# aws-neuron/neuronx-distributed-training

Measured on AMD Instinct MI355X. Metric: tokens_per_sec, higher is better.
Workload: dtype bf16; 1 GPU; model=llama3-8B, global_batch=4, seq_len=8192, parallelism=tp1_zero1

## Files before the change

neuronx_distributed_training_amd/ops/csrc/bindings.cpp:

```cpp
#include <torch/extension.h>

#include <hip/hip_runtime.h>

#include <c10/hip/HIPStream.h>

extern "C" {
void launch_rmsnorm_fwd(const void*, const void*, void*, void*, long, int,
                        float, hipStream_t);
void launch_rmsnorm_bwd(const void*, const void*, const void*, const void*,
                        void*, void*, long, int, hipStream_t);
void launch_swiglu_fwd(const void*, void*, long, int, hipStream_t);
void launch_swiglu_bwd(const void*, const void*, void*, long, int,
                       hipStream_t);
void launch_rope_fwd(const void*, const void*, const void*, void*, int, int,
                     int, int, const long*, int, int, float, hipStream_t);
void launch_adamw(void*, const void*, void*, void*, const void*, const void*,
                  void*, long, float, float, float, float, float, int,
                  hipStream_t);
void launch_flash_fwd(const void*, const void*, const void*, void*, void*,
                      int, int, int, int, int, int, bool, float, int,
                      const long*, const long*, const long*, hipStream_t);
void launch_flash_fwd_dbuf(const void*, const void*, const void*, void*,
                           void*, int, int, int, int, int, int, bool, float,
                           int, const long*, const long*, const long*,
                           hipStream_t);
void launch_flash_bwd(const void*, const void*, const void*, const void*,
                      const void*, const void*, void*, void*, void*, int, int,
                      int, int, int, int, bool, float, int, const long*,
                      const long*, const long*, const long*, hipStream_t);
void launch_attn_delta(const void*, const void*, void*, int, int, int, int,
                       const long*, const long*, hipStream_t);
void launch_flash_fwd_range(const void*, const void*, const void*, void*,
                            void*, int, int, int, int, int, int, bool, float,
                            int, const long*, const long*, const long*,
                            const int*, const int*, hipStream_t);
void launch_flash_bwd_range(const void*, const void*, const void*,
                            const void*, const void*, const void*, void*,
                            void*, void*, int, int, int, int, int, int, bool,
                            float, int, const long*, const long*, const long*,
                            const long*, const int*, const int*, hipStream_t);
void launch_flash_fwd_seg(const void*, const void*, const void*, void*, void*,
                          int, int, int, int, int, float, int, const long*,
                          const long*, const long*, const int*, const int*,
                          hipStream_t);
void launch_flash_bwd_seg(const void*, const void*, const void*, const void*,
                          const void*, const void*, void*, void*, void*, int,
                          int, int, int, int, float, int, const long*,
                          const long*, const long*, const long*, const int*,
                          const int*, hipStream_t);
void launch_mfma_probe(const void*, const void*, void*, hipStream_t);
void launch_mfma_probe32(const void*, const void*, void*, hipStream_t);
void launch_flash_fwd_v3(const void*, const void*, const void*, void*, void*,
                         int, int, int, int, int, bool, float, int,
                         const long*, const long*, const long*, hipStream_t);
void launch_flash_bwd_v3(const void*, const void*, const void*, const void*,
                         const void*, const void*, void*, void*, void*, int,
                         int, int, int, int, bool, float, int, const long*,
                         const long*, const long*, const long*, hipStream_t);
void launch_moe_gemm(const void*, const void*, void*, const int*, const int*,
                     int, int, int, long, bool, hipStream_t);
void launch_moe_wgrad(const void*, const void*, void*, const int*, int, int,
                      int, hipStream_t);
void launch_ce_fwd(const void*, const void*, void*, void*, void*, long, int,
                   long, hipStream_t);
void launch_ce_bwd(const void*, const void*, const void*, const void*,
                   const void*, void*, long, int, long, hipStream_t);
}

namespace {

hipStream_t cur_stream() {
  return c10::hip::getCurrentHIPStream().stream();
}

#define CHECK_IN(t)                                             \
  TORCH_CHECK((t).is_cuda(), #t " must be on GPU");             \
  TORCH_CHECK((t).is_contiguous(), #t " must be contiguous")

std::vector<torch::Tensor> rmsnorm_fwd(torch::Tensor x, torch::Tensor w,
                                       double eps) {
  CHECK_IN(x);
  CHECK_IN(w);
  TORCH_CHECK(x.scalar_type() == torch::kBFloat16, "rmsnorm: bf16 only");
  TORCH_CHECK(w.scalar_type() == torch::kBFloat16, "rmsnorm: w must be bf16");
  auto N = x.size(0);
  auto H = x.size(1);
  TORCH_CHECK(H % 8 == 0, "hidden must be divisible by 8");
  auto y = torch::empty_like(x);
  auto invrms = torch::empty({N}, x.options().dtype(torch::kFloat32));
  launch_rmsnorm_fwd(x.data_ptr(), w.data_ptr(), y.data_ptr(),
                     invrms.data_ptr(), N, (int)H, (float)eps, cur_stream());
  return {y, invrms};
}

std::vector<torch::Tensor> rmsnorm_bwd(torch::Tensor dy, torch::Tensor x,
                                       torch::Tensor w, torch::Tensor invrms) {
  CHECK_IN(dy);
  CHECK_IN(x);
  CHECK_IN(w);
  TORCH_CHECK(w.scalar_type() == torch::kBFloat16, "rmsnorm: w must be bf16");
  auto N = x.size(0);
  auto H = x.size(1);
  auto dx = torch::empty_like(x);
  auto dw32 = torch::zeros({H}, x.options().dtype(torch::kFloat32));
  launch_rmsnorm_bwd(dy.data_ptr(), x.data_ptr(), w.data_ptr(),
                     invrms.data_ptr(), dx.data_ptr(), dw32.data_ptr(), N,
                     (int)H, cur_stream());
  return {dx, dw32.to(w.scalar_type())};
}

torch::Tensor swiglu_fwd(torch::Tensor gu) {
  CHECK_IN(gu);
  auto N = gu.size(0);
  auto I = gu.size(1) / 2;
  TORCH_CHECK(I % 8 == 0, "intermediate must be divisible by 8");
  auto y = torch::empty({N, I}, gu.options());
  launch_swiglu_fwd(gu.data_ptr(), y.data_ptr(), N, (int)I, cur_stream());
  return y;
}

torch::Tensor swiglu_bwd(torch::Tensor dy, torch::Tensor gu) {
  CHECK_IN(dy);
  CHECK_IN(gu);
  auto N = gu.size(0);
  auto I = gu.size(1) / 2;
  auto dgu = torch::empty_like(gu);
  launch_swiglu_bwd(dy.data_ptr(), gu.data_ptr(), dgu.data_ptr(), N, (int)I,
                    cur_stream());
  return dgu;
}

torch::Tensor rope_fwd(torch::Tensor x, torch::Tensor cost, torch::Tensor sint,
                       long pos_offset, long pos_offset2) {
  TORCH_CHECK(x.is_cuda() && x.dim() == 4 && x.stride(3) == 1,
              "rope: x must be [b, h, s, d] on GPU with d contiguous");
  auto cos_c = cost.contiguous();
  auto sin_c = sint.contiguous();
  TORCH_CHECK(cos_c.scalar_type() == torch::kFloat32, "rope table must be f32");
  int B = (int)x.size(0), H = (int)x.size(1), S = (int)x.size(2),
      D = (int)x.size(3);
  TORCH_CHECK(pos_offset2 < 0 || S % 2 == 0, "zigzag rope needs even s");
  auto y_mem = torch::empty({S, B, H, D}, x.options());
  long xstr[3] = {x.stride(2), x.stride(0), x.stride(1)};
  launch_rope_fwd(x.data_ptr(), cos_c.data_ptr(), sin_c.data_ptr(),
                  y_mem.data_ptr(), S, B, H, D, xstr, (int)pos_offset,
                  (int)pos_offset2, 1.0f, cur_stream());
  return y_mem.permute({1, 2, 0, 3});
}

static void check_adamw_f32(const torch::Tensor& t, const torch::Tensor& p,
                            const char* name) {
  TORCH_CHECK(t.is_cuda() && t.device() == p.device(), "adamw: ", name,
              " must be on the same GPU as p");
  TORCH_CHECK(t.scalar_type() == torch::kFloat32, "adamw: ", name,
              " must be fp32");
  TORCH_CHECK(t.is_contiguous(), "adamw: ", name, " must be contiguous");
  TORCH_CHECK(t.numel() == p.numel(), "adamw: ", name,
              " must have p's numel");
  TORCH_CHECK(reinterpret_cast<uintptr_t>(t.data_ptr()) % 16 == 0, "adamw: ",
              name, " must be 16-byte aligned");
}

void adamw_step(torch::Tensor p, torch::Tensor g, torch::Tensor m,
                torch::Tensor v, torch::Tensor wd_mask, double lr, double b1,
                double b2, double eps, double wd, long step,
                c10::optional<torch::Tensor> grad_scale,
                c10::optional<torch::Tensor> p_bf16) {
  check_adamw_f32(p, p, "p");
  check_adamw_f32(g, p, "g");
  check_adamw_f32(m, p, "m");
  check_adamw_f32(v, p, "v");
  TORCH_CHECK(wd_mask.is_cuda() && wd_mask.device() == p.device(),
              "adamw: wd_mask must be on the same GPU as p");
  TORCH_CHECK(wd_mask.scalar_type() == torch::kBool,
              "adamw: wd_mask must be bool");
  TORCH_CHECK(wd_mask.is_contiguous() && wd_mask.numel() == p.numel(),
              "adamw: wd_mask must be contiguous with p's numel");
  TORCH_CHECK(step >= 1, "adamw: step must be >= 1");
  void* gs = nullptr;
  if (grad_scale.has_value()) {
    TORCH_CHECK(grad_scale->scalar_type() == torch::kFloat32 &&
                    grad_scale->is_cuda() &&
                    grad_scale->device() == p.device(),
                "grad_scale must be a device fp32 scalar");
    TORCH_CHECK(grad_scale->numel() == 1,
                "grad_scale must have exactly one element");
    gs = grad_scale->data_ptr();
  }
  void* pb = nullptr;
  if (p_bf16.has_value()) {
    TORCH_CHECK(p_bf16->is_cuda() && p_bf16->device() == p.device(),
                "adamw: p_bf16 must be on the same GPU as p");
    TORCH_CHECK(p_bf16->scalar_type() == torch::kBFloat16 &&
                    p_bf16->is_contiguous() && p_bf16->numel() == p.numel(),
                "p_bf16 must be contiguous bf16 of the same numel");
    TORCH_CHECK(reinterpret_cast<uintptr_t>(p_bf16->data_ptr()) % 8 == 0,
                "adamw: p_bf16 must be 8-byte aligned");
    pb = p_bf16->data_ptr();
  }
  launch_adamw(p.data_ptr(), g.data_ptr(), m.data_ptr(), v.data_ptr(),
               wd_mask.data_ptr(), gs, pb, p.numel(), (float)lr, (float)b1,
               (float)b2, (float)eps, (float)wd, (int)step, cur_stream());
}

static void check_bhsd(const torch::Tensor& t, const char* name) {
  TORCH_CHECK(t.is_cuda() && t.dim() == 4 && t.stride(3) == 1,
              name, " must be [b, h, s, d] on GPU with d contiguous");
  TORCH_CHECK(t.scalar_type() == torch::kBFloat16, name, " must be bf16");
}

static torch::Tensor check_bwd_args(const torch::Tensor& q,
                                    const torch::Tensor& k,
                                    const torch::Tensor& v,
                                    const torch::Tensor& lse) {
  check_bhsd(k, "k");
  check_bhsd(v, "v");
  TORCH_CHECK(q.size(3) == 128 || q.size(3) == 64,
              "head_dim must be 64 or 128");
  TORCH_CHECK(k.size(1) > 0 && q.size(1) % k.size(1) == 0,
              "GQA head mismatch");
  TORCH_CHECK(lse.is_cuda() && lse.device() == q.device(),
              "lse must be on the same GPU as q");
  TORCH_CHECK(lse.scalar_type() == torch::kFloat32, "lse must be fp32");
  TORCH_CHECK(lse.dim() == 3 && lse.size(0) == q.size(0) &&
                  lse.size(1) == q.size(1) && lse.size(2) == q.size(2),
              "lse must have shape [B, HQ, SQ]");
  return lse.contiguous();
}

static torch::Tensor attn_delta(torch::Tensor dout, torch::Tensor o) {
  auto oc = o.stride(3) == 1 ? o : o.contiguous();
  int B = (int)dout.size(0), HQ = (int)dout.size(1), SQ = (int)dout.size(2),
      D = (int)dout.size(3);
  auto delta = torch::empty(
      {B, HQ, SQ}, dout.options().dtype(torch::kFloat32));
  long ds[3] = {dout.stride(2), dout.stride(0), dout.stride(1)};
  long os_[3] = {oc.stride(2), oc.stride(0), oc.stride(1)};
  launch_attn_delta(dout.data_ptr(), oc.data_ptr(), delta.data_ptr(), SQ, B,
                    HQ, D, ds, os_, cur_stream());
  return delta;
}

std::vector<torch::Tensor> flash_attn_fwd_v3(torch::Tensor q, torch::Tensor k,
                                             torch::Tensor v, bool causal,
                                             double scale, long window) {
  check_bhsd(q, "q");
  check_bhsd(k, "k");
  check_bhsd(v, "v");
  int B = (int)q.size(0), HQ = (int)q.size(1), S = (int)q.size(2),
      D = (int)q.size(3);
  int HKV = (int)k.size(1);
  TORCH_CHECK(D == 128 || D == 64, "head_dim must be 64 or 128");
  TORCH_CHECK(k.size(2) == S, "v3 kernel requires S_q == S_kv (use v2)");
  auto o_mem = torch::empty({S, B, HQ, D}, q.options());
  auto lse = torch::empty({B, HQ, S}, q.options().dtype(torch::kFloat32));
  long qs[3] = {q.stride(2), q.stride(0), q.stride(1)};
  long ks[3] = {k.stride(2), k.stride(0), k.stride(1)};
  long vs[3] = {v.stride(2), v.stride(0), v.stride(1)};
  launch_flash_fwd_v3(q.data_ptr(), k.data_ptr(), v.data_ptr(),
                      o_mem.data_ptr(), lse.data_ptr(), B, HQ, HKV, S, D,
                      causal, (float)scale, (int)window, qs, ks, vs,
                      cur_stream());
  return {o_mem.permute({1, 2, 0, 3}), lse};
}

std::vector<torch::Tensor> flash_attn_bwd_v3(torch::Tensor dout,
                                             torch::Tensor q, torch::Tensor k,
                                             torch::Tensor v, torch::Tensor o,
                                             torch::Tensor lse, bool causal,
                                             double scale, long window) {
  if (dout.stride(3) != 1) dout = dout.contiguous();
  check_bhsd(dout, "dout");
  check_bhsd(q, "q");
  lse = check_bwd_args(q, k, v, lse);
  int B = (int)q.size(0), HQ = (int)q.size(1), S = (int)q.size(2),
      D = (int)q.size(3);
  int HKV = (int)k.size(1);
  TORCH_CHECK(k.size(2) == S, "v3 kernel requires S_q == S_kv (use v2)");
  auto delta = attn_delta(dout, o);
  auto dq_mem = torch::empty({S, B, HQ, D}, q.options());
  int group = HQ / HKV;
  auto f32 = q.options().dtype(torch::kFloat32);
  auto dk_part = torch::empty({group, S, B, HKV, D}, f32);
  auto dv_part = torch::empty({group, S, B, HKV, D}, f32);
  long qs[3] = {q.stride(2), q.stride(0), q.stride(1)};
  long ks[3] = {k.stride(2), k.stride(0), k.stride(1)};
  long vs[3] = {v.stride(2), v.stride(0), v.stride(1)};
  long dstr[3] = {dout.stride(2), dout.stride(0), dout.stride(1)};
  launch_flash_bwd_v3(dout.data_ptr(), q.data_ptr(), k.data_ptr(),
                      v.data_ptr(), lse.data_ptr(), delta.data_ptr(),
                      dq_mem.data_ptr(), dk_part.data_ptr(),
                      dv_part.data_ptr(), B, HQ, HKV, S, D, causal,
                      (float)scale, (int)window, qs, ks, vs, dstr,
                      cur_stream());
  auto dk_mem = dk_part.sum(0).to(torch::kBFloat16);
  auto dv_mem = dv_part.sum(0).to(torch::kBFloat16);
  return {dq_mem.permute({1, 2, 0, 3}), dk_mem.permute({1, 2, 0, 3}),
          dv_mem.permute({1, 2, 0, 3})};
}

std::vector<torch::Tensor> flash_attn_fwd(torch::Tensor q, torch::Tensor k,
                                          torch::Tensor v, bool causal,
                                          double scale, long window) {
  check_bhsd(q, "q");
  check_bhsd(k, "k");
  check_bhsd(v, "v");
  int B = (int)q.size(0), HQ = (int)q.size(1), SQ = (int)q.size(2),
      D = (int)q.size(3);
  int HKV = (int)k.size(1), SKV = (int)k.size(2);
  TORCH_CHECK(D == 128 || D == 64, "head_dim must be 64 or 128");
  TORCH_CHECK(HQ % HKV == 0, "GQA head mismatch");
  TORCH_CHECK(!causal || SKV >= SQ, "causal needs S_kv >= S_q");
  auto o_mem = torch::empty({SQ, B, HQ, D}, q.options());
  auto lse = torch::empty({B, HQ, SQ}, q.options().dtype(torch::kFloat32));
  long qs[3] = {q.stride(2), q.stride(0), q.stride(1)};
  long ks[3] = {k.stride(2), k.stride(0), k.stride(1)};
  long vs[3] = {v.stride(2), v.stride(0), v.stride(1)};
  launch_flash_fwd_dbuf(q.data_ptr(), k.data_ptr(), v.data_ptr(),
                        o_mem.data_ptr(), lse.data_ptr(), B, HQ, HKV, SQ,
                        SKV, D, causal, (float)scale, (int)window, qs, ks,
                        vs, cur_stream());
  return {o_mem.permute({1, 2, 0, 3}), lse};
}

std::vector<torch::Tensor> flash_attn_fwd_sbuf(torch::Tensor q,
                                               torch::Tensor k,
                                               torch::Tensor v, bool causal,
                                               double scale, long window) {
  check_bhsd(q, "q");
  check_bhsd(k, "k");
  check_bhsd(v, "v");
  int B = (int)q.size(0), HQ = (int)q.size(1), SQ = (int)q.size(2),
      D = (int)q.size(3);
  int HKV = (int)k.size(1), SKV = (int)k.size(2);
  TORCH_CHECK(D == 128 || D == 64, "head_dim must be 64 or 128");
  TORCH_CHECK(HQ % HKV == 0, "GQA head mismatch");
  TORCH_CHECK(!causal || SKV >= SQ, "causal needs S_kv >= S_q");
  auto o_mem = torch::empty({SQ, B, HQ, D}, q.options());
  auto lse = torch::empty({B, HQ, SQ}, q.options().dtype(torch::kFloat32));
  long qs[3] = {q.stride(2), q.stride(0), q.stride(1)};
  long ks[3] = {k.stride(2), k.stride(0), k.stride(1)};
  long vs[3] = {v.stride(2), v.stride(0), v.stride(1)};
  launch_flash_fwd(q.data_ptr(), k.data_ptr(), v.data_ptr(),
                        o_mem.data_ptr(), lse.data_ptr(), B, HQ, HKV, SQ,
                        SKV, D, causal, (float)scale, (int)window, qs, ks,
                        vs, cur_stream());
  return {o_mem.permute({1, 2, 0, 3}), lse};
}

std::vector<torch::Tensor> flash_attn_bwd(torch::Tensor dout, torch::Tensor q,
                                          torch::Tensor k, torch::Tensor v,
                                          torch::Tensor o, torch::Tensor lse,
                                          bool causal, double scale,
                                          long window) {
  if (dout.stride(3) != 1) dout = dout.contiguous();
  check_bhsd(dout, "dout");
  check_bhsd(q, "q");
  lse = check_bwd_args(q, k, v, lse);
  int B = (int)q.size(0), HQ = (int)q.size(1), SQ = (int)q.size(2),
      D = (int)q.size(3);
  int HKV = (int)k.size(1), SKV = (int)k.size(2);
  TORCH_CHECK(!causal || SKV >= SQ, "causal needs S_kv >= S_q");
  auto delta = attn_delta(dout, o);
  auto dq_mem = torch::empty({SQ, B, HQ, D}, q.options());
  int group = HQ / HKV;
  auto f32 = q.options().dtype(torch::kFloat32);
  auto dk_part = torch::empty({group, SKV, B, HKV, D}, f32);
  auto dv_part = torch::empty({group, SKV, B, HKV, D}, f32);
  long qs[3] = {q.stride(2), q.stride(0), q.stride(1)};
  long ks[3] = {k.stride(2), k.stride(0), k.stride(1)};
  long vs[3] = {v.stride(2), v.stride(0), v.stride(1)};
  long ds[3] = {dout.stride(2), dout.stride(0), dout.stride(1)};
  launch_flash_bwd(dout.data_ptr(), q.data_ptr(), k.data_ptr(), v.data_ptr(),
                   lse.data_ptr(), delta.data_ptr(), dq_mem.data_ptr(),
                   dk_part.data_ptr(), dv_part.data_ptr(), B, HQ, HKV, SQ,
                   SKV, D, causal, (float)scale, (int)window, qs, ks, vs, ds,
                   cur_stream());
  auto dk_mem = dk_part.sum(0).to(torch::kBFloat16);
  auto dv_mem = dv_part.sum(0).to(torch::kBFloat16);
  return {dq_mem.permute({1, 2, 0, 3}), dk_mem.permute({1, 2, 0, 3}),
          dv_mem.permute({1, 2, 0, 3})};
}

static void check_kv_range(const torch::Tensor& t, const torch::Tensor& q,
                           const char* name) {
  TORCH_CHECK(t.is_cuda() && t.device() == q.device(), name,
              " must be on the same GPU as q");
  TORCH_CHECK(t.scalar_type() == torch::kInt, name, " must be int32");
  TORCH_CHECK(t.dim() == 1 && t.size(0) == q.size(0), name,
              " must have shape [B]");
  TORCH_CHECK(t.is_contiguous(), name, " must be contiguous");
}

std::vector<torch::Tensor> flash_attn_fwd_range(
    torch::Tensor q, torch::Tensor k, torch::Tensor v, torch::Tensor kv_lo,
    torch::Tensor kv_hi, bool causal, double scale, long window) {
  check_bhsd(q, "q");
  check_bhsd(k, "k");
  check_bhsd(v, "v");
  check_kv_range(kv_lo, q, "kv_lo");
  check_kv_range(kv_hi, q, "kv_hi");
  int B = (int)q.size(0), HQ = (int)q.size(1), SQ = (int)q.size(2),
      D = (int)q.size(3);
  int HKV = (int)k.size(1), SKV = (int)k.size(2);
  TORCH_CHECK(D == 128 || D == 64, "head_dim must be 64 or 128");
  TORCH_CHECK(HQ % HKV == 0, "GQA head mismatch");
  TORCH_CHECK(!causal || SKV >= SQ, "causal needs S_kv >= S_q");
  auto o_mem = torch::empty({SQ, B, HQ, D}, q.options());
  auto lse = torch::empty({B, HQ, SQ}, q.options().dtype(torch::kFloat32));
  long qs[3] = {q.stride(2), q.stride(0), q.stride(1)};
  long ks[3] = {k.stride(2), k.stride(0), k.stride(1)};
  long vs[3] = {v.stride(2), v.stride(0), v.stride(1)};
  launch_flash_fwd_range(q.data_ptr(), k.data_ptr(), v.data_ptr(),
                         o_mem.data_ptr(), lse.data_ptr(), B, HQ, HKV, SQ,
                         SKV, D, causal, (float)scale, (int)window, qs, ks,
                         vs, kv_lo.data_ptr<int>(), kv_hi.data_ptr<int>(),
                         cur_stream());
  return {o_mem.permute({1, 2, 0, 3}), lse};
}

std::vector<torch::Tensor> flash_attn_bwd_range(
    torch::Tensor dout, torch::Tensor q, torch::Tensor k, torch::Tensor v,
    torch::Tensor o, torch::Tensor lse, torch::Tensor kv_lo,
    torch::Tensor kv_hi, bool causal, double scale, long window) {
  if (dout.stride(3) != 1) dout = dout.contiguous();
  check_bhsd(dout, "dout");
  check_bhsd(q, "q");
  lse = check_bwd_args(q, k, v, lse);
  check_kv_range(kv_lo, q, "kv_lo");
  check_kv_range(kv_hi, q, "kv_hi");
  int B = (int)q.size(0), HQ = (int)q.size(1), SQ = (int)q.size(2),
      D = (int)q.size(3);
  int HKV = (int)k.size(1), SKV = (int)k.size(2);
  TORCH_CHECK(!causal || SKV >= SQ, "causal needs S_kv >= S_q");
  auto delta = attn_delta(dout, o);
  auto dq_mem = torch::empty({SQ, B, HQ, D}, q.options());
  int group = HQ / HKV;
  auto f32 = q.options().dtype(torch::kFloat32);
  auto dk_part = torch::empty({group, SKV, B, HKV, D}, f32);
  auto dv_part = torch::empty({group, SKV, B, HKV, D}, f32);
  long qs[3] = {q.stride(2), q.stride(0), q.stride(1)};
  long ks[3] = {k.stride(2), k.stride(0), k.stride(1)};
  long vs[3] = {v.stride(2), v.stride(0), v.stride(1)};
  long ds[3] = {dout.stride(2), dout.stride(0), dout.stride(1)};
  launch_flash_bwd_range(dout.data_ptr(), q.data_ptr(), k.data_ptr(),
                         v.data_ptr(), lse.data_ptr(), delta.data_ptr(),
                         dq_mem.data_ptr(), dk_part.data_ptr(),
                         dv_part.data_ptr(), B, HQ, HKV, SQ, SKV, D, causal,
                         (float)scale, (int)window, qs, ks, vs, ds,
                         kv_lo.data_ptr<int>(), kv_hi.data_ptr<int>(),
                         cur_stream());
  auto dk_mem = dk_part.sum(0).to(torch::kBFloat16);
  auto dv_mem = dv_part.sum(0).to(torch::kBFloat16);
  return {dq_mem.permute({1, 2, 0, 3}), dk_mem.permute({1, 2, 0, 3}),
          dv_mem.permute({1, 2, 0, 3})};
}

static void check_seg_bound(const torch::Tensor& t, const torch::Tensor& q,
                            const char* name) {
  TORCH_CHECK(t.is_cuda() && t.device() == q.device(), name,
              " must be on the same GPU as q");
  TORCH_CHECK(t.scalar_type() == torch::kInt, name, " must be int32");
  TORCH_CHECK(t.dim() == 2 && t.size(0) == q.size(0) &&
                  t.size(1) == q.size(2),
              name, " must have shape [B, S]");
  TORCH_CHECK(t.is_contiguous(), name, " must be contiguous");
}

std::vector<torch::Tensor> flash_attn_fwd_seg(
    torch::Tensor q, torch::Tensor k, torch::Tensor v, torch::Tensor q_start,
    torch::Tensor k_end, double scale, long window) {
  check_bhsd(q, "q");
  check_bhsd(k, "k");
  check_bhsd(v, "v");
  int B = (int)q.size(0), HQ = (int)q.size(1), S = (int)q.size(2),
      D = (int)q.size(3);
  int HKV = (int)k.size(1);
  TORCH_CHECK(k.size(2) == S, "segmented attention needs S_q == S_kv");
  check_seg_bound(q_start, q, "q_start");
  check_seg_bound(k_end, q, "k_end");
  TORCH_CHECK(D == 128 || D == 64, "head_dim must be 64 or 128");
  TORCH_CHECK(HQ % HKV == 0, "GQA head mismatch");
  auto o_mem = torch::empty({S, B, HQ, D}, q.options());
  auto lse = torch::empty({B, HQ, S}, q.options().dtype(torch::kFloat32));
  long qs[3] = {q.stride(2), q.stride(0), q.stride(1)};
  long ks[3] = {k.stride(2), k.stride(0), k.stride(1)};
  long vs[3] = {v.stride(2), v.stride(0), v.stride(1)};
  launch_flash_fwd_seg(q.data_ptr(), k.data_ptr(), v.data_ptr(),
                       o_mem.data_ptr(), lse.data_ptr(), B, HQ, HKV, S, D,
                       (float)scale, (int)window, qs, ks, vs,
                       q_start.data_ptr<int>(), k_end.data_ptr<int>(),
                       cur_stream());
  return {o_mem.permute({1, 2, 0, 3}), lse};
}

std::vector<torch::Tensor> flash_attn_bwd_seg(
    torch::Tensor dout, torch::Tensor q, torch::Tensor k, torch::Tensor v,
    torch::Tensor o, torch::Tensor lse, torch::Tensor q_start,
    torch::Tensor k_end, double scale, long window) {
  if (dout.stride(3) != 1) dout = dout.contiguous();
  check_bhsd(dout, "dout");
  check_bhsd(q, "q");
  lse = check_bwd_args(q, k, v, lse);
  int B = (int)q.size(0), HQ = (int)q.size(1), S = (int)q.size(2),
      D = (int)q.size(3);
  int HKV = (int)k.size(1);
  TORCH_CHECK(k.size(2) == S, "segmented attention needs S_q == S_kv");
  check_seg_bound(q_start, q, "q_start");
  check_seg_bound(k_end, q, "k_end");
  auto delta = attn_delta(dout, o);
  auto dq_mem = torch::empty({S, B, HQ, D}, q.options());
  int group = HQ / HKV;
  auto f32 = q.options().dtype(torch::kFloat32);
  auto dk_part = torch::empty({group, S, B, HKV, D}, f32);
  auto dv_part = torch::empty({group, S, B, HKV, D}, f32);
  long qs[3] = {q.stride(2), q.stride(0), q.stride(1)};
  long ks[3] = {k.stride(2), k.stride(0), k.stride(1)};
  long vs[3] = {v.stride(2), v.stride(0), v.stride(1)};
  long ds[3] = {dout.stride(2), dout.stride(0), dout.stride(1)};
  launch_flash_bwd_seg(dout.data_ptr(), q.data_ptr(), k.data_ptr(),
                       v.data_ptr(), lse.data_ptr(), delta.data_ptr(),
                       dq_mem.data_ptr(), dk_part.data_ptr(),
                       dv_part.data_ptr(), B, HQ, HKV, S, D, (float)scale,
                       (int)window, qs, ks, vs, ds, q_start.data_ptr<int>(),
                       k_end.data_ptr<int>(), cur_stream());
  auto dk_mem = dk_part.sum(0).to(torch::kBFloat16);
  auto dv_mem = dv_part.sum(0).to(torch::kBFloat16);
  return {dq_mem.permute({1, 2, 0, 3}), dk_mem.permute({1, 2, 0, 3}),
          dv_mem.permute({1, 2, 0, 3})};
}

torch::Tensor moe_gemm(torch::Tensor a, torch::Tensor w,
                       torch::Tensor tile_expert, torch::Tensor total_rows,
                       bool trans_b) {
  CHECK_IN(a);
  CHECK_IN(w);
  CHECK_IN(tile_expert);
  CHECK_IN(total_rows);
  TORCH_CHECK(a.dim() == 2, "moe_gemm: a must be [Tp, K]");
  TORCH_CHECK(w.dim() == 3, "moe_gemm: w must be [E, N, Kw]");
  TORCH_CHECK(a.scalar_type() == torch::kBFloat16 &&
                  w.scalar_type() == torch::kBFloat16,
              "moe_gemm: bf16 only");
  TORCH_CHECK(tile_expert.scalar_type() == torch::kInt &&
                  total_rows.scalar_type() == torch::kInt,
              "moe_gemm: int32 maps");
  TORCH_CHECK(w.device() == a.device() && tile_expert.device() == a.device() &&
                  total_rows.device() == a.device(),
              "moe_gemm: w and the int32 maps must be on a's device");
  TORCH_CHECK(total_rows.numel() == 1, "moe_gemm: total_rows must be [1]");
  long Tp = a.size(0);
  int K = (int)a.size(1);
  int N = (int)w.size(1), Kw = (int)w.size(2);
  TORCH_CHECK(Tp % 256 == 0, "padded rows must be a multiple of 256");
  int row_tiles = (int)(Tp / 256);
  int contraction = trans_b ? N : Kw;
  int out_cols = trans_b ? Kw : N;
  TORCH_CHECK(K == contraction, "moe_gemm: contraction mismatch");
  TORCH_CHECK(K % 8 == 0, "moe_gemm: contraction % 8");
  TORCH_CHECK(out_cols % 128 == 0, "moe_gemm: out cols % 128");
  TORCH_CHECK(tile_expert.numel() >= row_tiles,
              "moe_gemm: tile_expert shorter than Tp / 256");
  auto c = torch::empty({Tp, out_cols}, a.options());
  launch_moe_gemm(a.data_ptr(), w.data_ptr(), c.data_ptr(),
                  tile_expert.data_ptr<int>(), total_rows.data_ptr<int>(),
                  row_tiles, K, out_cols, (long)N * Kw, trans_b,
                  cur_stream());
  return c;
}

torch::Tensor moe_wgrad(torch::Tensor dy, torch::Tensor x,
                        torch::Tensor seg_start, long E) {
  CHECK_IN(dy);
  CHECK_IN(x);
  CHECK_IN(seg_start);
  TORCH_CHECK(dy.dim() == 2 && x.dim() == 2,
              "moe_wgrad: dy must be [Tp, N] and x [Tp, K]");
  TORCH_CHECK(dy.scalar_type() == torch::kBFloat16 &&
                  x.scalar_type() == torch::kBFloat16,
              "moe_wgrad: bf16 only");
  TORCH_CHECK(seg_start.scalar_type() == torch::kInt, "int32 seg bounds");
  TORCH_CHECK(x.device() == dy.device() && seg_start.device() == dy.device(),
              "moe_wgrad: x and seg_start must be on dy's device");
  TORCH_CHECK(dy.size(0) == x.size(0), "moe_wgrad: dy and x row counts differ");
  TORCH_CHECK(dy.size(0) % 32 == 0, "moe_wgrad: rows % 32");
  TORCH_CHECK(E >= 1 && seg_start.numel() == E + 1,
              "moe_wgrad: seg_start must have E + 1 entries");
  int N = (int)dy.size(1), K = (int)x.size(1);
  TORCH_CHECK(N % 128 == 0 && K % 128 == 0, "moe_wgrad: dims % 128");
  auto dw = torch::empty({E, N, K}, dy.options().dtype(torch::kFloat32));
  launch_moe_wgrad(dy.data_ptr(), x.data_ptr(), dw.data_ptr(),
                   seg_start.data_ptr<int>(), (int)E, N, K, cur_stream());
  return dw;
}

torch::Tensor mfma_probe(torch::Tensor a, torch::Tensor b) {
  CHECK_IN(a);
  CHECK_IN(b);
  auto c = torch::empty({16, 16}, a.options().dtype(torch::kFloat32));
  launch_mfma_probe(a.data_ptr(), b.data_ptr(), c.data_ptr(), cur_stream());
  return c;
}

torch::Tensor mfma_probe32(torch::Tensor a, torch::Tensor b) {
  CHECK_IN(a);
  CHECK_IN(b);
  auto c = torch::empty({32, 32}, a.options().dtype(torch::kFloat32));
  launch_mfma_probe32(a.data_ptr(), b.data_ptr(), c.data_ptr(), cur_stream());
  return c;
}

std::vector<torch::Tensor> ce_fwd(torch::Tensor logits, torch::Tensor targets,
                                  long vocab_start) {
  CHECK_IN(logits);
  TORCH_CHECK(logits.scalar_type() == torch::kBFloat16, "ce: bf16 logits");
  TORCH_CHECK(targets.scalar_type() == torch::kLong, "ce: int64 targets");
  long N = logits.size(0);
  int V = (int)logits.size(1);
  auto opt = logits.options().dtype(torch::kFloat32);
  auto row_max = torch::empty({N}, opt);
  auto row_sumexp = torch::empty({N}, opt);
  auto tgt = torch::empty({N}, opt);
  launch_ce_fwd(logits.data_ptr(), targets.contiguous().data_ptr(),
                row_max.data_ptr(), row_sumexp.data_ptr(), tgt.data_ptr(), N,
                V, vocab_start, cur_stream());
  return {row_max, row_sumexp, tgt};
}

torch::Tensor ce_bwd(torch::Tensor logits, torch::Tensor targets,
                     torch::Tensor gmax, torch::Tensor gsum,
                     torch::Tensor gout, long vocab_start) {
  CHECK_IN(logits);
  long N = logits.size(0);
  int V = (int)logits.size(1);
  auto dl = torch::empty_like(logits);
  launch_ce_bwd(logits.data_ptr(), targets.contiguous().data_ptr(),
                gmax.contiguous().data_ptr(), gsum.contiguous().data_ptr(),
                gout.contiguous().data_ptr(), dl.data_ptr(), N, V,
                vocab_start, cur_stream());
  return dl;
}

}

PYBIND11_MODULE(TORCH_EXTENSION_NAME, m) {
  m.def("rmsnorm_fwd", &rmsnorm_fwd);
  m.def("rmsnorm_bwd", &rmsnorm_bwd);
  m.def("swiglu_fwd", &swiglu_fwd);
  m.def("swiglu_bwd", &swiglu_bwd);
  m.def("rope_fwd", &rope_fwd, py::arg("x"), py::arg("cost"), py::arg("sint"),
        py::arg("pos_offset"), py::arg("pos_offset2") = -1);
  m.def("adamw_step", &adamw_step, py::arg("p"), py::arg("g"), py::arg("m"),
        py::arg("v"), py::arg("wd_mask"), py::arg("lr"), py::arg("b1"),
        py::arg("b2"), py::arg("eps"), py::arg("wd"), py::arg("step"),
        py::arg("grad_scale") = py::none(), py::arg("p_bf16") = py::none());
  m.def("flash_attn_fwd_sbuf", &flash_attn_fwd_sbuf, pybind11::arg("q"),
        pybind11::arg("k"), pybind11::arg("v"), pybind11::arg("causal"),
        pybind11::arg("scale"), pybind11::arg("window") = 0);
  m.def("flash_attn_fwd", &flash_attn_fwd, pybind11::arg("q"),
        pybind11::arg("k"), pybind11::arg("v"), pybind11::arg("causal"),
        pybind11::arg("scale"), pybind11::arg("window") = 0);
  m.def("flash_attn_bwd", &flash_attn_bwd, pybind11::arg("dout"),
        pybind11::arg("q"), pybind11::arg("k"), pybind11::arg("v"),
        pybind11::arg("o"), pybind11::arg("lse"), pybind11::arg("causal"),
        pybind11::arg("scale"), pybind11::arg("window") = 0);
  m.def("flash_attn_fwd_range", &flash_attn_fwd_range, pybind11::arg("q"),
        pybind11::arg("k"), pybind11::arg("v"), pybind11::arg("kv_lo"),
        pybind11::arg("kv_hi"), pybind11::arg("causal"),
        pybind11::arg("scale"), pybind11::arg("window") = 0);
  m.def("flash_attn_bwd_range", &flash_attn_bwd_range, pybind11::arg("dout"),
        pybind11::arg("q"), pybind11::arg("k"), pybind11::arg("v"),
        pybind11::arg("o"), pybind11::arg("lse"), pybind11::arg("kv_lo"),
        pybind11::arg("kv_hi"), pybind11::arg("causal"),
        pybind11::arg("scale"), pybind11::arg("window") = 0);
  m.def("flash_attn_fwd_seg", &flash_attn_fwd_seg, pybind11::arg("q"),
        pybind11::arg("k"), pybind11::arg("v"), pybind11::arg("q_start"),
        pybind11::arg("k_end"), pybind11::arg("scale"),
        pybind11::arg("window") = 0);
  m.def("flash_attn_bwd_seg", &flash_attn_bwd_seg, pybind11::arg("dout"),
        pybind11::arg("q"), pybind11::arg("k"), pybind11::arg("v"),
        pybind11::arg("o"), pybind11::arg("lse"), pybind11::arg("q_start"),
        pybind11::arg("k_end"), pybind11::arg("scale"),
        pybind11::arg("window") = 0);
  m.def("mfma_probe", &mfma_probe);
  m.def("mfma_probe32", &mfma_probe32);
  m.def("flash_attn_fwd_v3", &flash_attn_fwd_v3, pybind11::arg("q"),
        pybind11::arg("k"), pybind11::arg("v"), pybind11::arg("causal"),
        pybind11::arg("scale"), pybind11::arg("window") = 0);
  m.def("flash_attn_bwd_v3", &flash_attn_bwd_v3, pybind11::arg("dout"),
        pybind11::arg("q"), pybind11::arg("k"), pybind11::arg("v"),
        pybind11::arg("o"), pybind11::arg("lse"), pybind11::arg("causal"),
        pybind11::arg("scale"), pybind11::arg("window") = 0);
  m.def("ce_fwd", &ce_fwd);
  m.def("ce_bwd", &ce_bwd);
  m.def("moe_gemm", &moe_gemm);
  m.def("moe_wgrad", &moe_wgrad);
}
```

neuronx_distributed_training_amd/ops/csrc/flash_attn_bwd.hip:

```cpp
#include "attn_common.h"

template <int D, bool CAUSAL, bool RANGED = false, bool SEGMENTED = false>
__global__ __launch_bounds__(512) void flash_bwd_dkv_kernel(
    const bf16* __restrict__ dO, const bf16* __restrict__ Q,
    const bf16* __restrict__ K, const bf16* __restrict__ V,
    const float* __restrict__ LSE, const float* __restrict__ DELTA,
    float* __restrict__ dK,
    float* __restrict__ dV,
    int SQ, int SKV, int Bb, int HQ, int HKV, float scale,
    int window, long sQs, long sQb, long sQh, long sKs, long sKb, long sKh,
    long sVs, long sVb, long sVh, long sDs, long sDb, long sDh,
    const int* __restrict__ kv_lo = nullptr,
    const int* __restrict__ kv_hi = nullptr) {
  static_assert(!(RANGED && SEGMENTED), "one mask mode at a time");
  static_assert(!SEGMENTED || CAUSAL, "segments are causal");
  constexpr int BN = 256;
  constexpr int BM = 64;
  const int coff = SKV - SQ;
  constexpr int KP = D + 8;
  constexpr int VP = BM + 8;
  __shared__ __bf16 q_lds[BM * KP];
  __shared__ __bf16 do_lds[BM * KP];
  __shared__ __bf16 dot_lds[D * VP];
  __shared__ __bf16 qt_lds[D * VP];
  __shared__ __bf16 pT_lds[8 * 32 * VP];
  __shared__ __bf16 dsT_lds[8 * 32 * VP];

  const int lane = threadIdx.x & 63;
  const int wid = threadIdx.x >> 6;
  const int group = HQ / HKV;
  int kblock, bhg;
  xcd_remap(kblock, bhg);
  const int g = bhg % group;
  const int hkv = (bhg / group) % HKV;
  const int b = bhg / (group * HKV);
  int lo = 0, hi = SKV;
  if constexpr (RANGED) {
    lo = kv_lo[b];
    hi = kv_hi[b];
  }

  const bf16* Kp = K + b * sKb + hkv * sKh;
  const bf16* Vp = V + b * sVb + hkv * sVh;
  const int kbase = kblock * BN;
  const int krow_w = kbase + wid * 32;

  constexpr int DK = D / 32;
  bf16x8_t kfrag[2][DK], vfrag[2][DK];
#pragma unroll
  for (int sb = 0; sb < 2; ++sb) {
    const int r = krow_w + sb * 16 + (lane & 15);
    const long row = (r < SKV) ? r : (SKV - 1);
#pragma unroll
    for (int kk = 0; kk < DK; ++kk) {
      *(int4*)&kfrag[sb][kk] =
          *(const int4*)(Kp + row * sKs + kk * 32 + (lane >> 4) * 8);
      *(int4*)&vfrag[sb][kk] =
          *(const int4*)(Vp + row * sVs + kk * 32 + (lane >> 4) * 8);
#pragma unroll
      for (int j = 0; j < 8; ++j)
        kfrag[sb][kk][j] = (__bf16)((float)kfrag[sb][kk][j] * scale);
    }
  }

  constexpr int DN2 = D / 32;
  f32x16_t dvacc[DN2], dkacc[DN2];
#pragma unroll
  for (int nj = 0; nj < DN2; ++nj) {
    dvacc[nj] = f32x16_t{};
    dkacc[nj] = f32x16_t{};
  }

  const int wkey_min = krow_w;

  {
    const int hq = hkv * group + g;
    const bf16* Qp = Q + b * sQb + hq * sQh;
    const bf16* dOp = dO + b * sDb + hq * sDh;
    const float* Lp = LSE + ((long)b * HQ + hq) * SQ;
    const float* Dp = DELTA + ((long)b * HQ + hq) * SQ;

    const int klo = RANGED ? max(kbase, lo) : kbase;
    const int khi = RANGED ? min(kbase + BN, hi) : kbase + BN;
    const int ib0 = CAUSAL ? max(0, (klo - coff) / BM) : 0;
    int nqb = (SQ + BM - 1) / BM;
    if (CAUSAL && window > 0)
      nqb = min(nqb, (khi - 1 + window - coff + BM - 1) / BM);
    if (RANGED && klo >= khi) nqb = 0;
    const int* Sp = kv_lo + (long)b * SQ;
    if constexpr (SEGMENTED)
      nqb = min(nqb,
                (kv_hi[(long)b * SQ + min(kbase + BN, SKV) - 1] + BM - 1) / BM);
    int qs_tile_next = 0;
    if constexpr (SEGMENTED)
      if (ib0 < nqb) qs_tile_next = Sp[ib0 * BM];
    for (int ib = ib0; ib < nqb; ++ib) {
      const int qbase = ib * BM;
      const int qs_tile = qs_tile_next;
      if constexpr (SEGMENTED)
        if (ib + 1 < nqb) qs_tile_next = Sp[qbase + BM];
      {
        constexpr int KVECS = BM * D / 8;
        for (int t = threadIdx.x; t < KVECS; t += 512) {
          const int row = t / (D / 8);
          const int col8 = (t % (D / 8)) * 8;
          const int gr = qbase + row;
          int4 qv = (gr < SQ) ? *(const int4*)(Qp + (long)gr * sQs + col8)
                              : int4{0, 0, 0, 0};
          int4 dv = (gr < SQ) ? *(const int4*)(dOp + (long)gr * sDs + col8)
                              : int4{0, 0, 0, 0};
          *(int4*)&q_lds[row * KP + col8] = qv;
          *(int4*)&do_lds[row * KP + col8] = dv;
        }
        constexpr int TVECS = BM * D / 16;
        for (int t = threadIdx.x; t < TVECS; t += 512) {
          const int row = (t / (D / 8)) * 2;
          const int col8 = (t % (D / 8)) * 8;
          const int g0 = qbase + row, g1 = g0 + 1;
          int4 q0 = (g0 < SQ) ? *(const int4*)(Qp + (long)g0 * sQs + col8)
                              : int4{0, 0, 0, 0};
          int4 q1 = (g1 < SQ) ? *(const int4*)(Qp + (long)g1 * sQs + col8)
                              : int4{0, 0, 0, 0};
          int4 d0 = (g0 < SQ) ? *(const int4*)(dOp + (long)g0 * sDs + col8)
                              : int4{0, 0, 0, 0};
          int4 d1 = (g1 < SQ) ? *(const int4*)(dOp + (long)g1 * sDs + col8)
                              : int4{0, 0, 0, 0};
          const __bf16 *qe0 = (const __bf16*)&q0, *qe1 = (const __bf16*)&q1;
          const __bf16 *de0 = (const __bf16*)&d0, *de1 = (const __bf16*)&d1;
#pragma unroll
          for (int j = 0; j < 8; ++j) {
            __bf16 qp[2] = {qe0[j], qe1[j]};
            __bf16 dp[2] = {de0[j], de1[j]};
            const int r = col8 + j;
            const uint byte = tr_swz((uint)(r * VP + row) * 2, r);
            *(uint*)((char*)qt_lds + byte) = *(uint*)qp;
            *(uint*)((char*)dot_lds + byte) = *(uint*)dp;
          }
        }
      }
      __syncthreads();

      if ((!CAUSAL || wkey_min <= qbase + BM - 1 + coff) &&
          (!RANGED || (krow_w < hi && krow_w + 32 > lo)) &&
          (!SEGMENTED || krow_w + 32 > qs_tile)) {
        __bf16* pw = &pT_lds[wid * 32 * VP];
        __bf16* dw = &dsT_lds[wid * 32 * VP];
#pragma unroll
        for (int nq = 0; nq < BM / 16; ++nq) {
          f32x4_t st[2], dpt[2];
          st[0] = st[1] = f32x4_t{0.f, 0.f, 0.f, 0.f};
          dpt[0] = dpt[1] = f32x4_t{0.f, 0.f, 0.f, 0.f};
#pragma unroll
          for (int kk = 0; kk < DK; ++kk) {
            bf16x8_t qb =
                load_frag_b_rowmajorT(&q_lds[nq * 16 * KP], KP, kk * 32, lane);
            st[0] = MFMA_16x16x32(kfrag[0][kk], qb, st[0]);
            st[1] = MFMA_16x16x32(kfrag[1][kk], qb, st[1]);
            bf16x8_t db =
                load_frag_b_rowmajorT(&do_lds[nq * 16 * KP], KP, kk * 32, lane);
            dpt[0] = MFMA_16x16x32(vfrag[0][kk], db, dpt[0]);
            dpt[1] = MFMA_16x16x32(vfrag[1][kk], db, dpt[1]);
          }
          const int qcol = qbase + nq * 16 + (lane & 15);
          const float lse = (qcol < SQ) ? Lp[qcol] : 1e30f;
          const float delta = (qcol < SQ) ? Dp[qcol] : 0.f;
          int qs = 0;
          if constexpr (SEGMENTED) qs = (qcol < SQ) ? Sp[qcol] : 0;
          const bool full_patch =
              (!RANGED || (krow_w >= lo && krow_w + 31 < hi)) &&
              (!SEGMENTED || krow_w >= __builtin_amdgcn_readlane(qs, 15)) &&
              (qbase + nq * 16 + 15 < SQ) && (krow_w + 31 < SKV) &&
              (!CAUSAL || (qbase + nq * 16 + coff >= krow_w + 31)) &&
              (window <= 0 ||
               (qbase + nq * 16 + 15 + coff < krow_w + window));
          if (full_patch) {
#pragma unroll
            for (int sb = 0; sb < 2; ++sb) {
#pragma unroll
              for (int r = 0; r < 4; ++r) {
                const float p = __expf(st[sb][r] - lse);
                const float ds = p * (dpt[sb][r] - delta) * scale;
                const int lrow = sb * 16 + (lane >> 4) * 4 + r;
                pw[lrow * VP + nq * 16 + (lane & 15)] = (__bf16)p;
                dw[lrow * VP + nq * 16 + (lane & 15)] = (__bf16)ds;
              }
            }
          } else {
#pragma unroll
            for (int sb = 0; sb < 2; ++sb) {
#pragma unroll
              for (int r = 0; r < 4; ++r) {
                const int krow = krow_w + sb * 16 + (lane >> 4) * 4 + r;
                bool dead = (qcol >= SQ) || (krow >= SKV) ||
                            (CAUSAL && qcol + coff < krow);
                if (CAUSAL && window > 0)
                  dead |= (qcol + coff >= krow + window);
                if constexpr (RANGED) dead |= (krow < lo) || (krow >= hi);
                if constexpr (SEGMENTED) dead |= (krow < qs);
                const float p = dead ? 0.f : __expf(st[sb][r] - lse);
                const float ds = p * (dpt[sb][r] - delta) * scale;
                const int lrow = sb * 16 + (lane >> 4) * 4 + r;
                pw[lrow * VP + nq * 16 + (lane & 15)] = (__bf16)p;
                dw[lrow * VP + nq * 16 + (lane & 15)] = (__bf16)ds;
              }
            }
          }
        }
#pragma unroll
        for (int kq = 0; kq < BM / 16; ++kq) {
          bf16x8_t pa = load_frag_a32(pw, VP, kq * 16, lane);
          bf16x8_t da = load_frag_a32(dw, VP, kq * 16, lane);
#pragma unroll
          for (int nj = 0; nj < DN2; ++nj) {
            bf16x8_t dob =
                load_frag_b32_trT_swz(dot_lds, VP, nj * 32, kq * 16, lane);
            dvacc[nj] = MFMA_32x32x16(pa, dob, dvacc[nj]);
            bf16x8_t qb2 =
                load_frag_b32_trT_swz(qt_lds, VP, nj * 32, kq * 16, lane);
            dkacc[nj] = MFMA_32x32x16(da, qb2, dkacc[nj]);
          }
        }
      }
      __syncthreads();
    }
  }

  const long sOs = (long)Bb * HKV * D;
  const long slab = (long)g * SKV * sOs + ((long)b * HKV + hkv) * D;
  float* dKp = dK + slab;
  float* dVp = dV + slab;
#pragma unroll
  for (int nj = 0; nj < DN2; ++nj) {
#pragma unroll
    for (int r = 0; r < 16; ++r) {
      const int krow = krow_w + (r & 3) + 8 * (r >> 2) + 4 * (lane >> 5);
      if (krow < SKV) {
        const int dcol = nj * 32 + (lane & 31);
        dKp[(long)krow * sOs + dcol] = dkacc[nj][r];
        dVp[(long)krow * sOs + dcol] = dvacc[nj][r];
      }
    }
  }
}

template <int D, bool CAUSAL, int NSB, bool RANGED = false,
          bool SEGMENTED = false>
__global__ __launch_bounds__(512) void flash_bwd_dq_kernel(
    const bf16* __restrict__ dO, const bf16* __restrict__ Q,
    const bf16* __restrict__ K, const bf16* __restrict__ V,
    const float* __restrict__ LSE, const float* __restrict__ DELTA,
    bf16* __restrict__ dQ,
    int SQ, int SKV, int Bb, int HQ, int HKV, float scale, int window,
    long sQs, long sQb, long sQh, long sKs, long sKb, long sKh, long sVs,
    long sVb, long sVh, long sDs, long sDb, long sDh,
    const int* __restrict__ kv_lo = nullptr,
    const int* __restrict__ kv_hi = nullptr) {
  static_assert(!(RANGED && SEGMENTED), "one mask mode at a time");
  static_assert(!SEGMENTED || CAUSAL, "segments are causal");
  constexpr int BM = NSB * 128, BN = 64;
  const int coff = SKV - SQ;
  constexpr int KP = D + 8;
  constexpr int VP = BN + 8;
  __shared__ __bf16 k_lds[2][BN * KP];
  __shared__ __bf16 v_lds[2][BN * KP];
  __shared__ __bf16 kt_lds[2][D * VP];
  __shared__ __bf16 ds_lds[8 * NSB * 16 * VP];

  const int lane = threadIdx.x & 63;
  const int wid = threadIdx.x >> 6;
  int qblock, bh;
  xcd_remap(qblock, bh);
  const int hq = bh % HQ;
  const int b = bh / HQ;
  const int hkv = hq / (HQ / HKV);
  int lo = 0, hi = SKV;
  if constexpr (RANGED) {
    lo = kv_lo[b];
    hi = kv_hi[b];
  }

  const bf16* Qp = Q + b * sQb + hq * sQh;
  const bf16* dOp = dO + b * sDb + hq * sDh;
  const bf16* Kp = K + b * sKb + hkv * sKh;
  const bf16* Vp = V + b * sVb + hkv * sVh;
  const float* Lp = LSE + ((long)b * HQ + hq) * SQ;
  const float* Dp = DELTA + ((long)b * HQ + hq) * SQ;

  const int q0 = qblock * BM;
  const int qrow_w = q0 + wid * NSB * 16;

  constexpr int DK = D / 32;
  bf16x8_t qfrag[NSB][DK], dofrag[NSB][DK];
  float lse[NSB][4], delta[NSB][4];
  int qs[NSB][4], qs_last = 0, qs_wave = 0;
  if constexpr (SEGMENTED) {
    const int* Sp = kv_lo + (long)b * SQ;
    qs_wave = Sp[min(qrow_w, SQ - 1)];
    qs_last = Sp[min(qrow_w + NSB * 16 - 1, SQ - 1)];
#pragma unroll
    for (int sb = 0; sb < NSB; ++sb)
#pragma unroll
      for (int rr = 0; rr < 4; ++rr)
        qs[sb][rr] = Sp[min(qrow_w + sb * 16 + (lane >> 4) * 4 + rr, SQ - 1)];
  }
#pragma unroll
  for (int sb = 0; sb < NSB; ++sb) {
    const int r = qrow_w + sb * 16 + (lane & 15);
    const long row = (r < SQ) ? r : (SQ - 1);
#pragma unroll
    for (int kk = 0; kk < DK; ++kk) {
      *(int4*)&qfrag[sb][kk] =
          *(const int4*)(Qp + row * sQs + kk * 32 + (lane >> 4) * 8);
      *(int4*)&dofrag[sb][kk] =
          *(const int4*)(dOp + row * sDs + kk * 32 + (lane >> 4) * 8);
#pragma unroll
      for (int j = 0; j < 8; ++j)
        qfrag[sb][kk][j] = (__bf16)((float)qfrag[sb][kk][j] * scale);
    }
#pragma unroll
    for (int rr = 0; rr < 4; ++rr) {
      const int qrow = qrow_w + sb * 16 + (lane >> 4) * 4 + rr;
      lse[sb][rr] = (qrow < SQ) ? Lp[qrow] : 1e30f;
      delta[sb][rr] = (qrow < SQ) ? Dp[qrow] : 0.f;
    }
  }

  constexpr int DN = D / 16;
  constexpr int DN2 = D / 32;
  f32x4_t dqacc[NSB == 1 ? NSB : 1][NSB == 1 ? DN : 1];
  f32x16_t dqacc32[NSB == 2 ? DN2 : 1];
  if constexpr (NSB == 1) {
#pragma unroll
    for (int sb = 0; sb < NSB; ++sb)
#pragma unroll
      for (int nj = 0; nj < DN; ++nj)
        dqacc[sb][nj] = f32x4_t{0.f, 0.f, 0.f, 0.f};
  } else {
#pragma unroll
    for (int nj = 0; nj < DN2; ++nj) dqacc32[nj] = f32x16_t{};
  }

  int kend = CAUSAL ? min(SKV, q0 + BM + coff) : SKV;
  if constexpr (RANGED) kend = min(kend, hi);
  const int nkb = (kend + BN - 1) / BN;
  int jb0 =
      (CAUSAL && window > 0) ? max(0, (q0 + coff - window + 1) / BN) : 0;
  if constexpr (RANGED) jb0 = max(jb0, lo / BN);
  if constexpr (SEGMENTED) jb0 = max(jb0, kv_lo[(long)b * SQ + q0] / BN);
  const int wrow_max = qrow_w + NSB * 16 - 1;

  auto stage_kv = [&](int jb, int buf) {
    const int kbase = jb * BN;
    constexpr int KVECS = BN * D / 8;
    for (int t = threadIdx.x; t < KVECS; t += 512) {
      const int row = t / (D / 8);
      const int col8 = (t % (D / 8)) * 8;
      const int gr = kbase + row;
      int4 kv = (gr < SKV) ? *(const int4*)(Kp + (long)gr * sKs + col8)
                           : int4{0, 0, 0, 0};
      int4 vv = (gr < SKV) ? *(const int4*)(Vp + (long)gr * sVs + col8)
                           : int4{0, 0, 0, 0};
      *(int4*)&k_lds[buf][row * KP + col8] = kv;
      *(int4*)&v_lds[buf][row * KP + col8] = vv;
    }
    constexpr int TVECS = BN * D / 16;
    for (int t = threadIdx.x; t < TVECS; t += 512) {
      const int row = (t / (D / 8)) * 2;
      const int col8 = (t % (D / 8)) * 8;
      const int g0 = kbase + row, g1 = g0 + 1;
      int4 k0 = (g0 < SKV) ? *(const int4*)(Kp + (long)g0 * sKs + col8)
                           : int4{0, 0, 0, 0};
      int4 k1 = (g1 < SKV) ? *(const int4*)(Kp + (long)g1 * sKs + col8)
                           : int4{0, 0, 0, 0};
      const __bf16 *e0 = (const __bf16*)&k0, *e1 = (const __bf16*)&k1;
#pragma unroll
      for (int j = 0; j < 8; ++j) {
        __bf16 pr[2] = {e0[j], e1[j]};
        const int r = col8 + j;
        *(uint*)((char*)kt_lds[buf] + tr_swz((uint)(r * VP + row) * 2, r)) =
            *(uint*)pr;
      }
    }
  };

  stage_kv(jb0, jb0 & 1);
  __syncthreads();

  for (int jb = jb0; jb < nkb; ++jb) {
    const int kbase = jb * BN;
    const int cur = jb & 1;
    if (jb + 1 < nkb) stage_kv(jb + 1, cur ^ 1);

    if ((!CAUSAL || kbase <= wrow_max + coff) &&
        (!SEGMENTED || kbase + BN > qs_wave)) {
      __bf16* dsw = &ds_lds[wid * NSB * 16 * VP];
#pragma unroll
      for (int nk = 0; nk < BN / 16; ++nk) {
        f32x4_t st[NSB], dpt[NSB];
#pragma unroll
        for (int sb = 0; sb < NSB; ++sb) {
          st[sb] = f32x4_t{0.f, 0.f, 0.f, 0.f};
          dpt[sb] = f32x4_t{0.f, 0.f, 0.f, 0.f};
        }
#pragma unroll
        for (int kk = 0; kk < DK; ++kk) {
          bf16x8_t kb = load_frag_b_rowmajorT(&k_lds[cur][nk * 16 * KP],
                                              KP, kk * 32, lane);
#pragma unroll
          for (int sb = 0; sb < NSB; ++sb)
            st[sb] = MFMA_16x16x32(qfrag[sb][kk], kb, st[sb]);
          bf16x8_t vb = load_frag_b_rowmajorT(&v_lds[cur][nk * 16 * KP],
                                              KP, kk * 32, lane);
#pragma unroll
          for (int sb = 0; sb < NSB; ++sb)
            dpt[sb] = MFMA_16x16x32(dofrag[sb][kk], vb, dpt[sb]);
        }
        const int kcol = kbase + nk * 16 + (lane & 15);
        const bool full_patch =
            (!RANGED ||
             (kbase + nk * 16 >= lo && kbase + nk * 16 + 15 < hi)) &&
            (!SEGMENTED || kbase + nk * 16 >= qs_last) &&
            (kbase + nk * 16 + 15 < SKV) &&
            (!CAUSAL || (kbase + nk * 16 + 15 <= qrow_w + coff)) &&
            (window <= 0 || (kbase + nk * 16 > qrow_w + 31 + coff - window));
        if (full_patch) {
#pragma unroll
          for (int sb = 0; sb < NSB; ++sb) {
#pragma unroll
            for (int r = 0; r < 4; ++r) {
              const float p = __expf(st[sb][r] - lse[sb][r]);
              const float ds = p * (dpt[sb][r] - delta[sb][r]) * scale;
              dsw[(sb * 16 + (lane >> 4) * 4 + r) * VP + nk * 16 +
                  (lane & 15)] = (__bf16)ds;
            }
          }
        } else {
#pragma unroll
          for (int sb = 0; sb < NSB; ++sb) {
#pragma unroll
            for (int r = 0; r < 4; ++r) {
              const int qrow = qrow_w + sb * 16 + (lane >> 4) * 4 + r;
              bool dead = (kcol >= SKV) || (CAUSAL && kcol > qrow + coff);
              if (CAUSAL && window > 0)
                dead |= (kcol <= qrow + coff - window);
              if constexpr (RANGED) dead |= (kcol < lo) || (kcol >= hi);
              if constexpr (SEGMENTED) dead |= (kcol < qs[sb][r]);
              const float p = dead ? 0.f : __expf(st[sb][r] - lse[sb][r]);
              const float ds = p * (dpt[sb][r] - delta[sb][r]) * scale;
              dsw[(sb * 16 + (lane >> 4) * 4 + r) * VP + nk * 16 +
                  (lane & 15)] = (__bf16)ds;
            }
          }
        }
      }
      if constexpr (NSB == 1) {
#pragma unroll
        for (int nj = 0; nj < DN; ++nj) {
#pragma unroll
          for (int kk = 0; kk < BN / 32; ++kk) {
            bf16x8_t kb2 =
                load_frag_b_trT_swz(kt_lds[cur], VP, nj * 16, kk * 32, lane);
            bf16x8_t da = load_frag_a(dsw, VP, kk * 32, lane);
            dqacc[0][nj] = MFMA_16x16x32(da, kb2, dqacc[0][nj]);
          }
        }
      } else {
#pragma unroll
        for (int kq = 0; kq < BN / 16; ++kq) {
          bf16x8_t da = load_frag_a32(dsw, VP, kq * 16, lane);
#pragma unroll
          for (int nj = 0; nj < DN2; ++nj) {
            bf16x8_t kb2 = load_frag_b32_trT_swz(kt_lds[cur], VP, nj * 32,
                                                 kq * 16, lane);
            dqacc32[nj] = MFMA_32x32x16(da, kb2, dqacc32[nj]);
          }
        }
      }
    }
    __syncthreads();
  }

  const long sOs = (long)Bb * HQ * D;
  bf16* dQp = dQ + ((long)b * HQ + hq) * D;
  if constexpr (NSB == 1) {
#pragma unroll
    for (int nj = 0; nj < DN; ++nj)
#pragma unroll
      for (int r = 0; r < 4; ++r) {
        const int qrow = qrow_w + (lane >> 4) * 4 + r;
        if (qrow < SQ)
          dQp[(long)qrow * sOs + nj * 16 + (lane & 15)] =
              f2bf(dqacc[0][nj][r]);
      }
  } else {
#pragma unroll
    for (int nj = 0; nj < DN2; ++nj)
#pragma unroll
      for (int r = 0; r < 16; ++r) {
        const int qrow = qrow_w + (r & 3) + 8 * (r >> 2) + 4 * (lane >> 5);
        if (qrow < SQ)
          dQp[(long)qrow * sOs + nj * 32 + (lane & 31)] =
              f2bf(dqacc32[nj][r]);
      }
  }
}

template <int D>
__global__ __launch_bounds__(256) void attn_delta_kernel(
    const bf16* __restrict__ dO, const bf16* __restrict__ O,
    float* __restrict__ DELTA, int SQ, int Bb, int HQ, long sDs, long sDb,
    long sDh, long sOs, long sOb, long sOh) {
  const int lane = threadIdx.x & 63;
  const long row = ((long)blockIdx.x * 4 + (threadIdx.x >> 6));
  const long total = (long)SQ * Bb * HQ;
  if (row >= total) return;
  const int s = (int)(row % SQ);
  const int h = (int)((row / SQ) % HQ);
  const int b = (int)(row / ((long)SQ * HQ));
  const bf16* dp = dO + b * sDb + h * sDh + s * sDs;
  const bf16* op = O + b * sOb + h * sOh + s * sOs;
  float acc = 0.f;
#pragma unroll
  for (int j = 0; j < D / 64; ++j) {
    const int c = lane + j * 64;
    acc += bf2f(dp[c]) * bf2f(op[c]);
  }
#pragma unroll
  for (int off = 1; off < 64; off <<= 1) acc += __shfl_xor(acc, off, 64);
  if (lane == 0) DELTA[row] = acc;
}

extern "C" {
void launch_attn_delta(const void* dout, const void* o, void* delta, int SQ,
                       int B, int HQ, int D, const long* dstr,
                       const long* ostr, hipStream_t stream) {
  long total = (long)SQ * B * HQ;
  dim3 grid((unsigned)((total + 3) / 4));
  dim3 blk(256);
  if (D == 128)
    attn_delta_kernel<128><<<grid, blk, 0, stream>>>(
        (const bf16*)dout, (const bf16*)o, (float*)delta, SQ, B, HQ, dstr[0],
        dstr[1], dstr[2], ostr[0], ostr[1], ostr[2]);
  else if (D == 64)
    attn_delta_kernel<64><<<grid, blk, 0, stream>>>(
        (const bf16*)dout, (const bf16*)o, (float*)delta, SQ, B, HQ, dstr[0],
        dstr[1], dstr[2], ostr[0], ostr[1], ostr[2]);
}

void launch_flash_bwd(const void* dout, const void* q, const void* k,
                      const void* v, const void* lse, const void* delta,
                      void* dq, void* dk, void* dv, int B, int HQ, int HKV,
                      int SQ, int SKV, int D, bool causal, float scale,
                      int window, const long* qstr, const long* kstr,
                      const long* vstr, const long* dostr,
                      hipStream_t stream) {
  dim3 blk(512);
  dim3 gkv((SKV + 255) / 256, B * HQ);
  const bool small = ((long)((SQ + 255) / 256) * B * HQ) < 512;
  const int bm = small ? 128 : 256;
  dim3 gq((SQ + bm - 1) / bm, B * HQ);
#define CASE(DD, CC)                                                          \
  do {                                                                        \
    flash_bwd_dkv_kernel<DD, CC><<<gkv, blk, 0, stream>>>(                    \
        (const bf16*)dout, (const bf16*)q, (const bf16*)k, (const bf16*)v,    \
        (const float*)lse, (const float*)delta, (float*)dk, (float*)dv, SQ,  \
        SKV, B, HQ, HKV, scale, window, qstr[0], qstr[1], qstr[2], kstr[0],   \
        kstr[1],                                                              \
        kstr[2], vstr[0], vstr[1], vstr[2], dostr[0], dostr[1], dostr[2]);    \
    if (small)                                                                \
      flash_bwd_dq_kernel<DD, CC, 1><<<gq, blk, 0, stream>>>(                 \
          (const bf16*)dout, (const bf16*)q, (const bf16*)k, (const bf16*)v,  \
          (const float*)lse, (const float*)delta, (bf16*)dq, SQ, SKV, B, HQ,  \
          HKV, scale, window, qstr[0], qstr[1], qstr[2], kstr[0], kstr[1],    \
          kstr[2], vstr[0], vstr[1], vstr[2], dostr[0], dostr[1], dostr[2]);  \
    else                                                                      \
      flash_bwd_dq_kernel<DD, CC, 2><<<gq, blk, 0, stream>>>(                 \
          (const bf16*)dout, (const bf16*)q, (const bf16*)k, (const bf16*)v,  \
          (const float*)lse, (const float*)delta, (bf16*)dq, SQ, SKV, B, HQ,  \
          HKV, scale, window, qstr[0], qstr[1], qstr[2], kstr[0], kstr[1],    \
          kstr[2], vstr[0], vstr[1], vstr[2], dostr[0], dostr[1], dostr[2]);  \
  } while (0)
  if (D == 128) {
    if (causal) CASE(128, true); else CASE(128, false);
  } else if (D == 64) {
    if (causal) CASE(64, true); else CASE(64, false);
  }
#undef CASE
}

void launch_flash_bwd_range(const void* dout, const void* q, const void* k,
                      const void* v, const void* lse, const void* delta,
                      void* dq, void* dk, void* dv, int B, int HQ, int HKV,
                      int SQ, int SKV, int D, bool causal, float scale,
                      int window, const long* qstr, const long* kstr,
                      const long* vstr, const long* dostr,
                      const int* kv_lo, const int* kv_hi,
                      hipStream_t stream) {
  dim3 blk(512);
  dim3 gkv((SKV + 255) / 256, B * HQ);
  const bool small = ((long)((SQ + 255) / 256) * B * HQ) < 512;
  const int bm = small ? 128 : 256;
  dim3 gq((SQ + bm - 1) / bm, B * HQ);
#define CASE(DD, CC)                                                          \
  do {                                                                        \
    flash_bwd_dkv_kernel<DD, CC, true><<<gkv, blk, 0, stream>>>(                    \
        (const bf16*)dout, (const bf16*)q, (const bf16*)k, (const bf16*)v,    \
        (const float*)lse, (const float*)delta, (float*)dk, (float*)dv, SQ,  \
        SKV, B, HQ, HKV, scale, window, qstr[0], qstr[1], qstr[2], kstr[0],   \
        kstr[1],                                                              \
        kstr[2], vstr[0], vstr[1], vstr[2], dostr[0], dostr[1], dostr[2],     \
        kv_lo, kv_hi);                                                        \
    if (small)                                                                \
      flash_bwd_dq_kernel<DD, CC, 1, true><<<gq, blk, 0, stream>>>(                 \
          (const bf16*)dout, (const bf16*)q, (const bf16*)k, (const bf16*)v,  \
          (const float*)lse, (const float*)delta, (bf16*)dq, SQ, SKV, B, HQ,  \
          HKV, scale, window, qstr[0], qstr[1], qstr[2], kstr[0], kstr[1],    \
          kstr[2], vstr[0], vstr[1], vstr[2], dostr[0], dostr[1], dostr[2],   \
          kv_lo, kv_hi);                                                      \
    else                                                                      \
      flash_bwd_dq_kernel<DD, CC, 2, true><<<gq, blk, 0, stream>>>(                 \
          (const bf16*)dout, (const bf16*)q, (const bf16*)k, (const bf16*)v,  \
          (const float*)lse, (const float*)delta, (bf16*)dq, SQ, SKV, B, HQ,  \
          HKV, scale, window, qstr[0], qstr[1], qstr[2], kstr[0], kstr[1],    \
          kstr[2], vstr[0], vstr[1], vstr[2], dostr[0], dostr[1], dostr[2],   \
          kv_lo, kv_hi);                                                      \
  } while (0)
  if (D == 128) {
    if (causal) CASE(128, true); else CASE(128, false);
  } else if (D == 64) {
    if (causal) CASE(64, true); else CASE(64, false);
  }
#undef CASE
}

void launch_flash_bwd_seg(const void* dout, const void* q, const void* k,
                      const void* v, const void* lse, const void* delta,
                      void* dq, void* dk, void* dv, int B, int HQ, int HKV,
                      int S, int D, float scale, int window,
                      const long* qstr, const long* kstr, const long* vstr,
                      const long* dostr, const int* q_start, const int* k_end,
                      hipStream_t stream) {
  dim3 blk(512);
  dim3 gkv((S + 255) / 256, B * HQ);
  const bool small = ((long)((S + 255) / 256) * B * HQ) < 512;
  const int bm = small ? 128 : 256;
  dim3 gq((S + bm - 1) / bm, B * HQ);
#define CASE(DD)                                                              \
  do {                                                                        \
    flash_bwd_dkv_kernel<DD, true, false, true><<<gkv, blk, 0, stream>>>(     \
        (const bf16*)dout, (const bf16*)q, (const bf16*)k, (const bf16*)v,    \
        (const float*)lse, (const float*)delta, (float*)dk, (float*)dv, S,   \
        S, B, HQ, HKV, scale, window, qstr[0], qstr[1], qstr[2], kstr[0],     \
        kstr[1],                                                              \
        kstr[2], vstr[0], vstr[1], vstr[2], dostr[0], dostr[1], dostr[2],     \
        q_start, k_end);                                                      \
    if (small)                                                                \
      flash_bwd_dq_kernel<DD, true, 1, false, true>                           \
          <<<gq, blk, 0, stream>>>(                                           \
          (const bf16*)dout, (const bf16*)q, (const bf16*)k, (const bf16*)v,  \
          (const float*)lse, (const float*)delta, (bf16*)dq, S, S, B, HQ,     \
          HKV, scale, window, qstr[0], qstr[1], qstr[2], kstr[0], kstr[1],    \
          kstr[2], vstr[0], vstr[1], vstr[2], dostr[0], dostr[1], dostr[2],   \
          q_start, k_end);                                                    \
    else                                                                      \
      flash_bwd_dq_kernel<DD, true, 2, false, true>                           \
          <<<gq, blk, 0, stream>>>(                                           \
          (const bf16*)dout, (const bf16*)q, (const bf16*)k, (const bf16*)v,  \
          (const float*)lse, (const float*)delta, (bf16*)dq, S, S, B, HQ,     \
          HKV, scale, window, qstr[0], qstr[1], qstr[2], kstr[0], kstr[1],    \
          kstr[2], vstr[0], vstr[1], vstr[2], dostr[0], dostr[1], dostr[2],   \
          q_start, k_end);                                                    \
  } while (0)
  if (D == 128) CASE(128);
  else if (D == 64) CASE(64);
#undef CASE
}
}
```

neuronx_distributed_training_amd/ops/flash_attn.py:

```python

from __future__ import annotations

import math
import os

import torch

from . import kernels_for


def _attn_version() -> str:
    env = os.environ.get("NXDT_ATTN_V3", "")
    if env == "1":
        return "3"
    if env == "fwd":
        return "fwd"
    return "2"


def _fwd_fn(kern, sq=None, skv=None):
    if _attn_version() in ("3", "fwd") and (sq is None or sq == skv):
        return kern.flash_attn_fwd_v3
    return kern.flash_attn_fwd


def _bwd_fn(kern, sq=None, skv=None):
    if _attn_version() == "3" and (sq is None or sq == skv):
        return kern.flash_attn_bwd_v3
    return kern.flash_attn_bwd


def mask_to_kv_range_tensors(attention_mask):
    m = attention_mask != 0
    s = m.size(1)
    mi = m.to(torch.int32)
    has = m.any(dim=1)
    lo = torch.argmax(mi, dim=1)
    hi = s - torch.argmax(mi.flip(1), dim=1)
    zero = torch.zeros_like(lo)
    lo = torch.where(has, lo, zero)
    hi = torch.where(has, hi, zero)
    contiguous = (mi.sum(dim=1) == hi - lo).all()
    return lo.to(torch.int32), hi.to(torch.int32), contiguous


def mask_to_kv_range(attention_mask):
    lo, hi, contiguous = mask_to_kv_range_tensors(attention_mask)
    return lo, hi, bool(contiguous)


def _norm_kv_range(kv_range, b, skv, device):
    lo, hi = kv_range
    lo = torch.as_tensor(lo, device=device).to(torch.int32).reshape(-1)
    hi = torch.as_tensor(hi, device=device).to(torch.int32).reshape(-1)
    if lo.numel() != b or hi.numel() != b:
        raise ValueError(
            f"kv_range tensors must have shape [{b}], got "
            f"{tuple(lo.shape)} / {tuple(hi.shape)}"
        )
    hi = hi.clamp(0, skv)
    lo = torch.minimum(lo.clamp(0, skv), hi)
    return lo.contiguous(), hi.contiguous()


def segment_bounds(segment_ids):
    if segment_ids.dim() != 2:
        raise ValueError(
            f"segment_ids must be [B, S], got {tuple(segment_ids.shape)}"
        )
    b, s = segment_ids.shape
    pos = torch.arange(s, device=segment_ids.device, dtype=torch.int32)
    pos = pos.expand(b, s)
    new = torch.ones(b, s, dtype=torch.bool, device=segment_ids.device)
    new[:, 1:] = segment_ids[:, 1:] != segment_ids[:, :-1]
    q_start = torch.cummax(torch.where(new, pos, torch.zeros_like(pos)),
                           dim=1).values
    last = torch.ones_like(new)
    last[:, :-1] = new[:, 1:]
    end = torch.where(last, pos + 1, torch.full_like(pos, s))
    k_end = torch.cummin(end.flip(1), dim=1).values.flip(1)
    return (q_start.to(torch.int32).contiguous(),
            k_end.to(torch.int32).contiguous())


def _make_mask(sq, sk, causal, window, device, kv_lo=None, kv_hi=None,
               q_start=None):
    mask = torch.zeros(sq, sk, dtype=torch.bool, device=device)
    if causal:
        diag = sk - sq
        mask |= torch.ones(sq, sk, dtype=torch.bool, device=device).triu(
            1 + diag
        )
        if window and window > 0:
            mask |= torch.ones(sq, sk, dtype=torch.bool, device=device).tril(
                diag - window
            )
    if kv_lo is not None:
        j = torch.arange(sk, device=device)
        out = (j[None, :] < kv_lo[:, None]) | (j[None, :] >= kv_hi[:, None])
        mask = mask[None, None] | out[:, None, None, :]
    if q_start is not None:
        j = torch.arange(sk, device=device)
        out = j[None, None, :] < q_start[:, :, None]
        mask = mask[None, None] | out[:, None]
    return mask


def _ranged_softmax(s, mask):
    s = s.masked_fill(mask, float("-inf"))
    m = s.amax(dim=-1, keepdim=True)
    empty = torch.isinf(m)
    m = torch.where(empty, torch.zeros_like(m), m)
    e = torch.exp(s - m)
    l = e.sum(dim=-1, keepdim=True)
    p = e / torch.where(empty, torch.ones_like(l), l)
    lse = torch.where(empty, torch.full_like(m, -1e30), m + torch.log(l))
    return p, lse.squeeze(-1)


def _cpu_ref_fwd(q, k, v, causal, scale, window=0, kv_lo=None, kv_hi=None,
                 q_start=None):
    hq, hkv = q.size(1), k.size(1)
    if hq != hkv:
        k = k.repeat_interleave(hq // hkv, dim=1)
        v = v.repeat_interleave(hq // hkv, dim=1)
    qf, kf, vf = q.float(), k.float(), v.float()
    s = torch.matmul(qf, kf.transpose(-1, -2)) * scale
    mask = _make_mask(q.size(-2), k.size(-2), causal, window, q.device,
                      kv_lo, kv_hi, q_start)
    if kv_lo is not None:
        p, lse = _ranged_softmax(s, mask)
    else:
        s = s.masked_fill(mask, float("-inf"))
        lse = torch.logsumexp(s, dim=-1)
        p = torch.softmax(s, dim=-1)
    o = torch.matmul(p, vf)
    return o.to(q.dtype), lse


class _FlashAttnFn(torch.autograd.Function):
    @staticmethod
    def forward(ctx, q, k, v, causal: bool, scale: float, window: int = 0,
                kv_lo=None, kv_hi=None, q_start=None, k_end=None):
        kern = kernels_for(q)
        ranged = kv_lo is not None
        segmented = q_start is not None
        if kern is not None and segmented:
            o, lse = kern.flash_attn_fwd_seg(
                q, k, v, q_start, k_end, scale, window
            )
        elif kern is not None and ranged:
            o, lse = kern.flash_attn_fwd_range(
                q, k, v, kv_lo, kv_hi, causal, scale, window
            )
        elif kern is not None:
            o, lse = _fwd_fn(kern, q.size(2), k.size(2))(
                q, k, v, causal, scale, window
            )
        else:
            o, lse = _cpu_ref_fwd(q, k, v, causal, scale, window,
                                  kv_lo, kv_hi, q_start)
        if segmented:
            ctx.save_for_backward(q, k, v, o, lse, q_start, k_end)
        elif ranged:
            ctx.save_for_backward(q, k, v, o, lse, kv_lo, kv_hi)
        else:
            ctx.save_for_backward(q, k, v, o, lse)
        ctx.ranged = ranged
        ctx.segmented = segmented
        ctx.causal = causal
        ctx.scale = scale
        ctx.window = window
        return o

    @staticmethod
    def backward(ctx, do):
        kv_lo = kv_hi = q_start = k_end = None
        none7 = (None,) * 7
        if ctx.segmented:
            q, k, v, o, lse, q_start, k_end = ctx.saved_tensors
        elif ctx.ranged:
            q, k, v, o, lse, kv_lo, kv_hi = ctx.saved_tensors
        else:
            q, k, v, o, lse = ctx.saved_tensors
        kern = kernels_for(q)
        if kern is not None and ctx.segmented:
            dq, dk, dv = kern.flash_attn_bwd_seg(
                do, q, k, v, o, lse, q_start, k_end, ctx.scale, ctx.window
            )
            return (dq, dk, dv) + none7
        if kern is not None and ctx.ranged:
            dq, dk, dv = kern.flash_attn_bwd_range(
                do, q, k, v, o, lse, kv_lo, kv_hi, ctx.causal, ctx.scale,
                ctx.window,
            )
            return (dq, dk, dv) + none7
        if kern is not None:
            dq, dk, dv = _bwd_fn(kern, q.size(2), k.size(2))(
                do, q, k, v, o, lse, ctx.causal, ctx.scale, ctx.window
            )
            return (dq, dk, dv) + none7
        hq, hkv = q.size(1), k.size(1)
        g = hq // hkv
        kx = k.repeat_interleave(g, dim=1).float()
        vx = v.repeat_interleave(g, dim=1).float()
        qf, dof = q.float(), do.float()
        s = torch.matmul(qf, kx.transpose(-1, -2)) * ctx.scale
        mask = _make_mask(q.size(-2), k.size(-2), ctx.causal, ctx.window,
                          q.device, kv_lo, kv_hi, q_start)
        if ctx.ranged:
            p, _ = _ranged_softmax(s, mask)
        else:
            s = s.masked_fill(mask, float("-inf"))
            p = torch.softmax(s, dim=-1)
        dv = torch.matmul(p.transpose(-1, -2), dof)
        dp = torch.matmul(dof, vx.transpose(-1, -2))
        delta = (dof * o.float()).sum(-1, keepdim=True)
        ds = p * (dp - delta) * ctx.scale
        dq = torch.matmul(ds, kx)
        dk = torch.matmul(ds.transpose(-1, -2), qf)
        if g > 1:
            dk = dk.reshape(dk.size(0), hkv, g, dk.size(-2), dk.size(-1)).sum(2)
            dv = dv.reshape(dv.size(0), hkv, g, dv.size(-2), dv.size(-1)).sum(2)
        return (dq.to(q.dtype), dk.to(k.dtype), dv.to(v.dtype)) + none7


def flash_attn_func(
    q: torch.Tensor,
    k: torch.Tensor,
    v: torch.Tensor,
    causal: bool = True,
    scale: float | None = None,
    window: int | None = None,
    kv_range=None,
    segment_ids=None,
    seg_bounds=None,
) -> torch.Tensor:
    if scale is None:
        scale = 1.0 / math.sqrt(q.size(-1))
    if segment_ids is not None or seg_bounds is not None:
        if segment_ids is not None and seg_bounds is not None:
            raise ValueError("give segment_ids or seg_bounds, not both")
        if kv_range is not None:
            raise ValueError("segment_ids and kv_range are mutually exclusive")
        if not causal:
            raise ValueError("segment_ids needs causal=True")
        if q.size(2) != k.size(2):
            raise ValueError(
                f"segment_ids needs S_q == S_kv, got {q.size(2)} / {k.size(2)}"
            )
        if seg_bounds is None:
            seg_bounds = segment_bounds(
                torch.as_tensor(segment_ids, device=q.device)
            )
        q_start, k_end = seg_bounds
        want = (q.size(0), q.size(2))
        if tuple(q_start.shape) != want or tuple(k_end.shape) != want:
            raise ValueError(
                f"segment_ids must have shape {list(want)}, got "
                f"{tuple(q_start.shape)}"
            )
        return _FlashAttnFn.apply(
            q, k, v, True, scale, int(window or 0), None, None,
            q_start, k_end,
        )
    if kv_range is None:
        return _FlashAttnFn.apply(q, k, v, causal, scale, int(window or 0))
    kv_lo, kv_hi = _norm_kv_range(kv_range, q.size(0), k.size(2), q.device)
    return _FlashAttnFn.apply(
        q, k, v, causal, scale, int(window or 0), kv_lo, kv_hi
    )
```

neuronx_distributed_training_amd/ops/ring_attn.py:

```python

from __future__ import annotations

import math
from typing import List

import torch
import torch.distributed as dist

from ..parallel import state as ps
from .flash_attn import _FlashAttnFn, _cpu_ref_fwd, _make_mask
from . import kernels_for


def _neighbors():
    ring = ps.get_context_model_parallel_ring_ranks()
    me = ps.get_context_model_parallel_rank()
    return ring[(me + 1) % len(ring)], ring[(me - 1) % len(ring)]


def _post_shift(send_tensors, recv_buffers):
    nxt, prv = _neighbors()
    group = ps.get_context_model_parallel_group()
    ops = []
    for t in send_tensors:
        ops.append(dist.P2POp(dist.isend, t, nxt, group=group))
    for b in recv_buffers:
        ops.append(dist.P2POp(dist.irecv, b, prv, group=group))
    return dist.batch_isend_irecv(ops)


def _fwd_block(kern, q, k, v, causal, scale):
    if kern is not None:
        o, lse = kern.flash_attn_fwd(q, k, v, causal, scale)
        return o, lse
    return _cpu_ref_fwd(q, k, v, causal, scale)


def _merge_into(acc_o, acc_lse, o, lse):
    new_lse = torch.logaddexp(acc_lse, lse)
    acc_o.mul_(torch.exp(acc_lse - new_lse).unsqueeze(-1))
    acc_o.add_(o.float() * torch.exp(lse - new_lse).unsqueeze(-1))
    acc_lse.copy_(new_lse)


def _cpu_block_bwd(do, q, k, v, out, lse, causal, scale):
    hq, hkv = q.size(1), k.size(1)
    g = hq // hkv
    kx = k.repeat_interleave(g, 1).float()
    vx = v.repeat_interleave(g, 1).float()
    qf, dof = q.float(), do.float()
    s = torch.matmul(qf, kx.transpose(-1, -2)) * scale
    if causal:
        mask = _make_mask(q.size(-2), k.size(-2), True, 0, q.device)
        s = s.masked_fill(mask, float("-inf"))
    p = torch.exp(s - lse.unsqueeze(-1))
    dv = torch.matmul(p.transpose(-1, -2), dof)
    dp = torch.matmul(dof, vx.transpose(-1, -2))
    delta = (dof * out.float()).sum(-1, keepdim=True)
    ds = p * (dp - delta) * scale
    dq = torch.matmul(ds, kx)
    dk = torch.matmul(ds.transpose(-1, -2), qf)
    if g > 1:
        dk = dk.reshape(dk.size(0), hkv, g, dk.size(-2), dk.size(-1)).sum(2)
        dv = dv.reshape(dv.size(0), hkv, g, dv.size(-2), dv.size(-1)).sum(2)
    return dq.to(q.dtype), dk.to(k.dtype), dv.to(v.dtype)


def _bwd_block(kern, do, q, k, v, out, lse, causal, scale):
    if kern is not None:
        return kern.flash_attn_bwd(
            do.contiguous(), q, k, v, out, lse, causal, scale
        )
    return _cpu_block_bwd(do, q, k, v, out, lse, causal, scale)


def _ring_fwd_hop(kern, r, j, q, k_blk, v_blk, acc_o, acc_lse, scale):
    half = q.size(2) // 2
    if j == r:
        o, lse = _fwd_block(kern, q, k_blk, v_blk, True, scale)
        _merge_into(acc_o, acc_lse, o, lse)
    elif j < r:
        o, lse = _fwd_block(
            kern, q, k_blk[:, :, :half], v_blk[:, :, :half], False, scale,
        )
        _merge_into(acc_o, acc_lse, o, lse)
    else:
        o, lse = _fwd_block(kern, q[:, :, half:], k_blk, v_blk, False, scale)
        _merge_into(acc_o[:, :, half:], acc_lse[:, :, half:], o, lse)


def _ring_bwd_hop(kern, r, j, dout, q, k_blk, v_blk, out, lse, dq_acc, scale):
    half = q.size(2) // 2
    lo_only = j < r
    if j == r:
        dq_j, dk_j, dv_j = _bwd_block(
            kern, dout, q, k_blk, v_blk, out, lse, True, scale
        )
        dq_acc += dq_j
    elif j < r:
        dq_j, dk_j, dv_j = _bwd_block(
            kern, dout, q, k_blk[:, :, :half], v_blk[:, :, :half],
            out, lse, False, scale,
        )
        dq_acc += dq_j
    else:
        dq_j, dk_j, dv_j = _bwd_block(
            kern, dout[:, :, half:], q[:, :, half:], k_blk, v_blk,
            out[:, :, half:], lse[:, :, half:], False, scale,
        )
        dq_acc[:, :, half:] += dq_j
    return dk_j, dv_j, lo_only


class _RingFlashAttnFn(torch.autograd.Function):
    @staticmethod
    def forward(ctx, q, k, v, scale):
        R = ps.get_context_model_parallel_world_size()
        r = ps.get_context_model_parallel_rank()
        kern = kernels_for(q)
        s_loc = q.size(2)
        assert s_loc % 2 == 0, "zigzag CP needs an even local sequence"
        k_cur, v_cur = k.contiguous(), v.contiguous()
        k_bufs = [torch.empty_like(k_cur), torch.empty_like(k_cur)]
        v_bufs = [torch.empty_like(v_cur), torch.empty_like(v_cur)]

        acc_o = torch.zeros(q.shape, dtype=torch.float32, device=q.device)
        acc_lse = torch.full(
            (q.size(0), q.size(1), s_loc), -1e30,
            dtype=torch.float32, device=q.device,
        )
        with torch.no_grad():
            for t in range(R):
                j = (r - t) % R
                works: List = []
                if t < R - 1:
                    works = _post_shift(
                        (k_cur, v_cur), (k_bufs[t % 2], v_bufs[t % 2])
                    )
                _ring_fwd_hop(
                    kern, r, j, q, k_cur, v_cur, acc_o, acc_lse, scale
                )
                for w in works:
                    w.wait()
                if t < R - 1:
                    k_cur, v_cur = k_bufs[t % 2], v_bufs[t % 2]
            out = acc_o.to(q.dtype)
        ctx.save_for_backward(q, k, v, out, acc_lse)
        ctx.scale = scale
        return out

    @staticmethod
    def backward(ctx, dout):
        q, k, v, out, lse = ctx.saved_tensors
        scale = ctx.scale
        R = ps.get_context_model_parallel_world_size()
        r = ps.get_context_model_parallel_rank()
        kern = kernels_for(q)
        half = q.size(2) // 2
        dout = dout.contiguous()
        out = out.contiguous()
        k_cur, v_cur = k.contiguous(), v.contiguous()
        k_bufs = [torch.empty_like(k_cur), torch.empty_like(k_cur)]
        v_bufs = [torch.empty_like(v_cur), torch.empty_like(v_cur)]
        dk_cur = torch.zeros_like(k_cur)
        dv_cur = torch.zeros_like(v_cur)
        dk_buf = torch.empty_like(dk_cur)
        dv_buf = torch.empty_like(dv_cur)
        dq_acc = torch.zeros_like(q)

        acc_works: List = []
        for t in range(R):
            j = (r - t) % R
            kv_works: List = []
            if t < R - 1:
                kv_works = _post_shift(
                    (k_cur, v_cur), (k_bufs[t % 2], v_bufs[t % 2])
                )
            dk_j, dv_j, lo_only = _ring_bwd_hop(
                kern, r, j, dout, q, k_cur, v_cur, out, lse, dq_acc, scale
            )
            for w in acc_works:
                w.wait()
            if t > 0:
                dk_cur, dk_buf = dk_buf, dk_cur
                dv_cur, dv_buf = dv_buf, dv_cur
            if lo_only:
                dk_cur[:, :, :half].add_(dk_j)
                dv_cur[:, :, :half].add_(dv_j)
            else:
                dk_cur.add_(dk_j)
                dv_cur.add_(dv_j)
            acc_works = _post_shift((dk_cur, dv_cur), (dk_buf, dv_buf))
            for w in kv_works:
                w.wait()
            if t < R - 1:
                k_cur, v_cur = k_bufs[t % 2], v_bufs[t % 2]
        for w in acc_works:
            w.wait()
        return dq_acc, dk_buf, dv_buf, None


def ring_flash_attn(
    q: torch.Tensor, k: torch.Tensor, v: torch.Tensor, scale: float = None
) -> torch.Tensor:
    if scale is None:
        scale = 1.0 / math.sqrt(q.size(-1))
    if ps.get_context_model_parallel_world_size() == 1:
        return _FlashAttnFn.apply(q, k, v, True, scale)
    return _RingFlashAttnFn.apply(q, k, v, scale)
```

setup.py:

```python

import os

from setuptools import setup

os.environ.setdefault("PYTORCH_ROCM_ARCH", "gfx950")

from torch.utils.cpp_extension import BuildExtension, CUDAExtension

HERE = os.path.dirname(os.path.abspath(__file__))
CSRC = os.path.join(HERE, "neuronx_distributed_training_amd", "ops", "csrc")

sources = [
    os.path.join(CSRC, f)
    for f in (
        "bindings.cpp",
        "rmsnorm.hip",
        "swiglu.hip",
        "rope.hip",
        "adamw.hip",
        "flash_attn_fwd.hip",
        "flash_attn_fwd_dbuf.hip",
        "flash_attn_fwd_v3.hip",
        "flash_attn_bwd_v3.hip",
        "flash_attn_bwd.hip",
        "cross_entropy.hip",
        "moe_gemm.hip",
        "probe.hip",
    )
]

import pybind11
from setuptools import Extension

setup(
    name="neuronx_distributed_training_amd_ext",
    ext_modules=[
        CUDAExtension(
            name="neuronx_distributed_training_amd.ops._C",
            sources=sources,
            extra_compile_args={
                "cxx": ["-O3", "-std=c++17"],
                "nvcc": ["-O3", "-std=c++17", "--offload-arch=gfx950"],
            },
        ),
        Extension(
            name="neuronx_distributed_training_amd.data._helpers_cpp",
            sources=[
                os.path.join(
                    HERE, "neuronx_distributed_training_amd", "data",
                    "csrc_cpu", "helpers.cpp",
                )
            ],
            include_dirs=[pybind11.get_include()],
            extra_compile_args=["-O3", "-std=c++17"],
            language="c++",
        ),
    ],
    cmdclass={"build_ext": BuildExtension.with_options(use_ninja=True)},
)
```

Before: 15780 tokens/s.

## Add pipelined dK/dV flash-attention backward kernel and make it the default

Adds a new dK/dV backward kernel for v2 flash attention that software-pipelines tile loads into LDS. It builds P and dS fragments in LDS and accumulates with 32x32x16 MFMAs, reading the transposed operands with a swizzled layout. One templated kernel covers the plain, ranged and segmented variants. The bindings are consolidated into a shared helper exposing pipe and `_sbuf` variants, selected by the NXDT_ATTN_DKV env var (default pipe). The aim is to hide global-memory latency in the dK/dV pass; the cost is a new stride limit below 2^24 elements and more code to keep correct.

```diff
diff --git a/neuronx_distributed_training_amd/ops/csrc/bindings.cpp b/neuronx_distributed_training_amd/ops/csrc/bindings.cpp
--- a/neuronx_distributed_training_amd/ops/csrc/bindings.cpp
+++ b/neuronx_distributed_training_amd/ops/csrc/bindings.cpp
@@ -27,7 +27,8 @@
 void launch_flash_bwd(const void*, const void*, const void*, const void*,
                       const void*, const void*, void*, void*, void*, int, int,
                       int, int, int, int, bool, float, int, const long*,
-                      const long*, const long*, const long*, hipStream_t);
+                      const long*, const long*, const long*, bool,
+                      hipStream_t);
 void launch_attn_delta(const void*, const void*, void*, int, int, int, int,
                        const long*, const long*, hipStream_t);
 void launch_flash_fwd_range(const void*, const void*, const void*, void*,
@@ -38,7 +39,8 @@
                             const void*, const void*, const void*, void*,
                             void*, void*, int, int, int, int, int, int, bool,
                             float, int, const long*, const long*, const long*,
-                            const long*, const int*, const int*, hipStream_t);
+                            const long*, const int*, const int*, bool,
+                            hipStream_t);
 void launch_flash_fwd_seg(const void*, const void*, const void*, void*, void*,
                           int, int, int, int, int, float, int, const long*,
                           const long*, const long*, const int*, const int*,
@@ -47,7 +49,7 @@
                           const void*, const void*, void*, void*, void*, int,
                           int, int, int, int, float, int, const long*,
                           const long*, const long*, const long*, const int*,
-                          const int*, hipStream_t);
+                          const int*, bool, hipStream_t);
 void launch_mfma_probe(const void*, const void*, void*, hipStream_t);
 void launch_mfma_probe32(const void*, const void*, void*, hipStream_t);
 void launch_flash_fwd_v3(const void*, const void*, const void*, void*, void*,
@@ -348,40 +350,6 @@
   return {o_mem.permute({1, 2, 0, 3}), lse};
 }
 
-std::vector<torch::Tensor> flash_attn_bwd(torch::Tensor dout, torch::Tensor q,
-                                          torch::Tensor k, torch::Tensor v,
-                                          torch::Tensor o, torch::Tensor lse,
-                                          bool causal, double scale,
-                                          long window) {
-  if (dout.stride(3) != 1) dout = dout.contiguous();
-  check_bhsd(dout, "dout");
-  check_bhsd(q, "q");
-  lse = check_bwd_args(q, k, v, lse);
-  int B = (int)q.size(0), HQ = (int)q.size(1), SQ = (int)q.size(2),
-      D = (int)q.size(3);
-  int HKV = (int)k.size(1), SKV = (int)k.size(2);
-  TORCH_CHECK(!causal || SKV >= SQ, "causal needs S_kv >= S_q");
-  auto delta = attn_delta(dout, o);
-  auto dq_mem = torch::empty({SQ, B, HQ, D}, q.options());
-  int group = HQ / HKV;
-  auto f32 = q.options().dtype(torch::kFloat32);
-  auto dk_part = torch::empty({group, SKV, B, HKV, D}, f32);
-  auto dv_part = torch::empty({group, SKV, B, HKV, D}, f32);
-  long qs[3] = {q.stride(2), q.stride(0), q.stride(1)};
-  long ks[3] = {k.stride(2), k.stride(0), k.stride(1)};
-  long vs[3] = {v.stride(2), v.stride(0), v.stride(1)};
-  long ds[3] = {dout.stride(2), dout.stride(0), dout.stride(1)};
-  launch_flash_bwd(dout.data_ptr(), q.data_ptr(), k.data_ptr(), v.data_ptr(),
-                   lse.data_ptr(), delta.data_ptr(), dq_mem.data_ptr(),
-                   dk_part.data_ptr(), dv_part.data_ptr(), B, HQ, HKV, SQ,
-                   SKV, D, causal, (float)scale, (int)window, qs, ks, vs, ds,
-                   cur_stream());
-  auto dk_mem = dk_part.sum(0).to(torch::kBFloat16);
-  auto dv_mem = dv_part.sum(0).to(torch::kBFloat16);
-  return {dq_mem.permute({1, 2, 0, 3}), dk_mem.permute({1, 2, 0, 3}),
-          dv_mem.permute({1, 2, 0, 3})};
-}
-
 static void check_kv_range(const torch::Tensor& t, const torch::Tensor& q,
                            const char* name) {
   TORCH_CHECK(t.is_cuda() && t.device() == q.device(), name,
@@ -419,43 +387,6 @@
   return {o_mem.permute({1, 2, 0, 3}), lse};
 }
 
-std::vector<torch::Tensor> flash_attn_bwd_range(
-    torch::Tensor dout, torch::Tensor q, torch::Tensor k, torch::Tensor v,
-    torch::Tensor o, torch::Tensor lse, torch::Tensor kv_lo,
-    torch::Tensor kv_hi, bool causal, double scale, long window) {
-  if (dout.stride(3) != 1) dout = dout.contiguous();
-  check_bhsd(dout, "dout");
-  check_bhsd(q, "q");
-  lse = check_bwd_args(q, k, v, lse);
-  check_kv_range(kv_lo, q, "kv_lo");
-  check_kv_range(kv_hi, q, "kv_hi");
-  int B = (int)q.size(0), HQ = (int)q.size(1), SQ = (int)q.size(2),
-      D = (int)q.size(3);
-  int HKV = (int)k.size(1), SKV = (int)k.size(2);
-  TORCH_CHECK(!causal || SKV >= SQ, "causal needs S_kv >= S_q");
-  auto delta = attn_delta(dout, o);
-  auto dq_mem = torch::empty({SQ, B, HQ, D}, q.options());
-  int group = HQ / HKV;
-  auto f32 = q.options().dtype(torch::kFloat32);
-  auto dk_part = torch::empty({group, SKV, B, HKV, D}, f32);
-  auto dv_part = torch::empty({group, SKV, B, HKV, D}, f32);
-  long qs[3] = {q.stride(2), q.stride(0), q.stride(1)};
-  long ks[3] = {k.stride(2), k.stride(0), k.stride(1)};
-  long vs[3] = {v.stride(2), v.stride(0), v.stride(1)};
-  long ds[3] = {dout.stride(2), dout.stride(0), dout.stride(1)};
-  launch_flash_bwd_range(dout.data_ptr(), q.data_ptr(), k.data_ptr(),
-                         v.data_ptr(), lse.data_ptr(), delta.data_ptr(),
-                         dq_mem.data_ptr(), dk_part.data_ptr(),
-                         dv_part.data_ptr(), B, HQ, HKV, SQ, SKV, D, causal,
-                         (float)scale, (int)window, qs, ks, vs, ds,
-                         kv_lo.data_ptr<int>(), kv_hi.data_ptr<int>(),
-                         cur_stream());
-  auto dk_mem = dk_part.sum(0).to(torch::kBFloat16);
-  auto dv_mem = dv_part.sum(0).to(torch::kBFloat16);
-  return {dq_mem.permute({1, 2, 0, 3}), dk_mem.permute({1, 2, 0, 3}),
-          dv_mem.permute({1, 2, 0, 3})};
-}
-
 static void check_seg_bound(const torch::Tensor& t, const torch::Tensor& q,
                             const char* name) {
   TORCH_CHECK(t.is_cuda() && t.device() == q.device(), name,
@@ -494,41 +425,94 @@
   return {o_mem.permute({1, 2, 0, 3}), lse};
 }
 
-std::vector<torch::Tensor> flash_attn_bwd_seg(
-    torch::Tensor dout, torch::Tensor q, torch::Tensor k, torch::Tensor v,
-    torch::Tensor o, torch::Tensor lse, torch::Tensor q_start,
-    torch::Tensor k_end, double scale, long window) {
+static std::vector<torch::Tensor> flash_bwd_common(
+    int mode, bool pipe, torch::Tensor dout, torch::Tensor q, torch::Tensor k,
+    torch::Tensor v, torch::Tensor o, torch::Tensor lse, const torch::Tensor* a,
+    const torch::Tensor* b, bool causal, double scale, long window) {
   if (dout.stride(3) != 1) dout = dout.contiguous();
   check_bhsd(dout, "dout");
   check_bhsd(q, "q");
   lse = check_bwd_args(q, k, v, lse);
-  int B = (int)q.size(0), HQ = (int)q.size(1), S = (int)q.size(2),
+  int B = (int)q.size(0), HQ = (int)q.size(1), SQ = (int)q.size(2),
       D = (int)q.size(3);
-  int HKV = (int)k.size(1);
-  TORCH_CHECK(k.size(2) == S, "segmented attention needs S_q == S_kv");
-  check_seg_bound(q_start, q, "q_start");
-  check_seg_bound(k_end, q, "k_end");
+  int HKV = (int)k.size(1), SKV = (int)k.size(2);
+  if (mode == 1) {
+    check_kv_range(*a, q, "kv_lo");
+    check_kv_range(*b, q, "kv_hi");
+  }
+  if (mode == 2) {
+    TORCH_CHECK(SKV == SQ, "segmented attention needs S_q == S_kv");
+    check_seg_bound(*a, q, "q_start");
+    check_seg_bound(*b, q, "k_end");
+  } else {
+    TORCH_CHECK(!causal || SKV >= SQ, "causal needs S_kv >= S_q");
+  }
+  TORCH_CHECK(!pipe || (q.stride(2) >= 0 && q.stride(2) < (1L << 24) &&
+                        dout.stride(2) >= 0 && dout.stride(2) < (1L << 24)),
+              "q / dout sequence stride must be below 2^24 elements");
   auto delta = attn_delta(dout, o);
-  auto dq_mem = torch::empty({S, B, HQ, D}, q.options());
+  auto dq_mem = torch::empty({SQ, B, HQ, D}, q.options());
   int group = HQ / HKV;
   auto f32 = q.options().dtype(torch::kFloat32);
-  auto dk_part = torch::empty({group, S, B, HKV, D}, f32);
-  auto dv_part = torch::empty({group, S, B, HKV, D}, f32);
+  auto dk_part = torch::empty({group, SKV, B, HKV, D}, f32);
+  auto dv_part = torch::empty({group, SKV, B, HKV, D}, f32);
   long qs[3] = {q.stride(2), q.stride(0), q.stride(1)};
   long ks[3] = {k.stride(2), k.stride(0), k.stride(1)};
   long vs[3] = {v.stride(2), v.stride(0), v.stride(1)};
   long ds[3] = {dout.stride(2), dout.stride(0), dout.stride(1)};
-  launch_flash_bwd_seg(dout.data_ptr(), q.data_ptr(), k.data_ptr(),
-                       v.data_ptr(), lse.data_ptr(), delta.data_ptr(),
-                       dq_mem.data_ptr(), dk_part.data_ptr(),
-                       dv_part.data_ptr(), B, HQ, HKV, S, D, (float)scale,
-                       (int)window, qs, ks, vs, ds, q_start.data_ptr<int>(),
-                       k_end.data_ptr<int>(), cur_stream());
+  if (mode == 0)
+    launch_flash_bwd(dout.data_ptr(), q.data_ptr(), k.data_ptr(),
+                     v.data_ptr(), lse.data_ptr(), delta.data_ptr(),
+                     dq_mem.data_ptr(), dk_part.data_ptr(),
+                     dv_part.data_ptr(), B, HQ, HKV, SQ, SKV, D, causal,
+                     (float)scale, (int)window, qs, ks, vs, ds, pipe,
+                     cur_stream());
+  else if (mode == 1)
+    launch_flash_bwd_range(dout.data_ptr(), q.data_ptr(), k.data_ptr(),
+                           v.data_ptr(), lse.data_ptr(), delta.data_ptr(),
+                           dq_mem.data_ptr(), dk_part.data_ptr(),
+                           dv_part.data_ptr(), B, HQ, HKV, SQ, SKV, D, causal,
+                           (float)scale, (int)window, qs, ks, vs, ds,
+                           a->data_ptr<int>(), b->data_ptr<int>(), pipe,
+                           cur_stream());
+  else
+    launch_flash_bwd_seg(dout.data_ptr(), q.data_ptr(), k.data_ptr(),
+                         v.data_ptr(), lse.data_ptr(), delta.data_ptr(),
+                         dq_mem.data_ptr(), dk_part.data_ptr(),
+                         dv_part.data_ptr(), B, HQ, HKV, SQ, D, (float)scale,
+                         (int)window, qs, ks, vs, ds, a->data_ptr<int>(),
+                         b->data_ptr<int>(), pipe, cur_stream());
   auto dk_mem = dk_part.sum(0).to(torch::kBFloat16);
   auto dv_mem = dv_part.sum(0).to(torch::kBFloat16);
   return {dq_mem.permute({1, 2, 0, 3}), dk_mem.permute({1, 2, 0, 3}),
           dv_mem.permute({1, 2, 0, 3})};
 }
+
+#define BWD_BINDINGS(SUFFIX, PIPE)                                            \
+  std::vector<torch::Tensor> flash_attn_bwd##SUFFIX(                          \
+      torch::Tensor dout, torch::Tensor q, torch::Tensor k, torch::Tensor v,  \
+      torch::Tensor o, torch::Tensor lse, bool causal, double scale,          \
+      long window) {                                                          \
+    return flash_bwd_common(0, PIPE, dout, q, k, v, o, lse, nullptr, nullptr, \
+                            causal, scale, window);                           \
+  }                                                                           \
+  std::vector<torch::Tensor> flash_attn_bwd_range##SUFFIX(                    \
+      torch::Tensor dout, torch::Tensor q, torch::Tensor k, torch::Tensor v,  \
+      torch::Tensor o, torch::Tensor lse, torch::Tensor kv_lo,                \
+      torch::Tensor kv_hi, bool causal, double scale, long window) {          \
+    return flash_bwd_common(1, PIPE, dout, q, k, v, o, lse, &kv_lo, &kv_hi,   \
+                            causal, scale, window);                           \
+  }                                                                           \
+  std::vector<torch::Tensor> flash_attn_bwd_seg##SUFFIX(                      \
+      torch::Tensor dout, torch::Tensor q, torch::Tensor k, torch::Tensor v,  \
+      torch::Tensor o, torch::Tensor lse, torch::Tensor q_start,              \
+      torch::Tensor k_end, double scale, long window) {                       \
+    return flash_bwd_common(2, PIPE, dout, q, k, v, o, lse, &q_start, &k_end, \
+                            true, scale, window);                             \
+  }
+BWD_BINDINGS(, true)
+BWD_BINDINGS(_sbuf, false)
+#undef BWD_BINDINGS
 
 torch::Tensor moe_gemm(torch::Tensor a, torch::Tensor w,
                        torch::Tensor tile_expert, torch::Tensor total_rows,
@@ -682,6 +666,21 @@
         pybind11::arg("o"), pybind11::arg("lse"), pybind11::arg("q_start"),
         pybind11::arg("k_end"), pybind11::arg("scale"),
         pybind11::arg("window") = 0);
+  m.def("flash_attn_bwd_sbuf", &flash_attn_bwd_sbuf, pybind11::arg("dout"),
+        pybind11::arg("q"), pybind11::arg("k"), pybind11::arg("v"),
+        pybind11::arg("o"), pybind11::arg("lse"), pybind11::arg("causal"),
+        pybind11::arg("scale"), pybind11::arg("window") = 0);
+  m.def("flash_attn_bwd_range_sbuf", &flash_attn_bwd_range_sbuf,
+        pybind11::arg("dout"), pybind11::arg("q"), pybind11::arg("k"),
+        pybind11::arg("v"), pybind11::arg("o"), pybind11::arg("lse"),
+        pybind11::arg("kv_lo"), pybind11::arg("kv_hi"),
+        pybind11::arg("causal"), pybind11::arg("scale"),
+        pybind11::arg("window") = 0);
+  m.def("flash_attn_bwd_seg_sbuf", &flash_attn_bwd_seg_sbuf,
+        pybind11::arg("dout"), pybind11::arg("q"), pybind11::arg("k"),
+        pybind11::arg("v"), pybind11::arg("o"), pybind11::arg("lse"),
+        pybind11::arg("q_start"), pybind11::arg("k_end"),
+        pybind11::arg("scale"), pybind11::arg("window") = 0);
   m.def("mfma_probe", &mfma_probe);
   m.def("mfma_probe32", &mfma_probe32);
   m.def("flash_attn_fwd_v3", &flash_attn_fwd_v3, pybind11::arg("q"),
diff --git a/neuronx_distributed_training_amd/ops/csrc/flash_attn_bwd.hip b/neuronx_distributed_training_amd/ops/csrc/flash_attn_bwd.hip
--- a/neuronx_distributed_training_amd/ops/csrc/flash_attn_bwd.hip
+++ b/neuronx_distributed_training_amd/ops/csrc/flash_attn_bwd.hip
@@ -547,13 +547,26 @@
         dstr[1], dstr[2], ostr[0], ostr[1], ostr[2]);
 }
 
+void launch_flash_dkv_pipe(const void* dout, const void* q, const void* k,
+                           const void* v, const void* lse, const void* delta,
+                           void* dk, void* dv, int B, int HQ, int HKV, int SQ,
+                           int SKV, int D, bool causal, float scale,
+                           int window, const long* qstr, const long* kstr,
+                           const long* vstr, const long* dostr, int mode,
+                           const int* bound_a, const int* bound_b,
+                           hipStream_t stream);
+
 void launch_flash_bwd(const void* dout, const void* q, const void* k,
                       const void* v, const void* lse, const void* delta,
                       void* dq, void* dk, void* dv, int B, int HQ, int HKV,
                       int SQ, int SKV, int D, bool causal, float scale,
                       int window, const long* qstr, const long* kstr,
-                      const long* vstr, const long* dostr,
+                      const long* vstr, const long* dostr, bool pipe,
                       hipStream_t stream) {
+  if (pipe)
+    launch_flash_dkv_pipe(dout, q, k, v, lse, delta, dk, dv, B, HQ, HKV, SQ,
+                          SKV, D, causal, scale, window, qstr, kstr, vstr,
+                          dostr, 0, nullptr, nullptr, stream);
   dim3 blk(512);
   dim3 gkv((SKV + 255) / 256, B * HQ);
   const bool small = ((long)((SQ + 255) / 256) * B * HQ) < 512;
@@ -561,6 +574,7 @@
   dim3 gq((SQ + bm - 1) / bm, B * HQ);
 #define CASE(DD, CC)                                                          \
   do {                                                                        \
+    if (!pipe)                                                                \
     flash_bwd_dkv_kernel<DD, CC><<<gkv, blk, 0, stream>>>(                    \
         (const bf16*)dout, (const bf16*)q, (const bf16*)k, (const bf16*)v,    \
         (const float*)lse, (const float*)delta, (float*)dk, (float*)dv, SQ,  \
@@ -594,8 +608,12 @@
                       int SQ, int SKV, int D, bool causal, float scale,
                       int window, const long* qstr, const long* kstr,
                       const long* vstr, const long* dostr,
-                      const int* kv_lo, const int* kv_hi,
+                      const int* kv_lo, const int* kv_hi, bool pipe,
                       hipStream_t stream) {
+  if (pipe)
+    launch_flash_dkv_pipe(dout, q, k, v, lse, delta, dk, dv, B, HQ, HKV, SQ,
+                          SKV, D, causal, scale, window, qstr, kstr, vstr,
+                          dostr, 1, kv_lo, kv_hi, stream);
   dim3 blk(512);
   dim3 gkv((SKV + 255) / 256, B * HQ);
   const bool small = ((long)((SQ + 255) / 256) * B * HQ) < 512;
@@ -603,6 +621,7 @@
   dim3 gq((SQ + bm - 1) / bm, B * HQ);
 #define CASE(DD, CC)                                                          \
   do {                                                                        \
+    if (!pipe)                                                                \
     flash_bwd_dkv_kernel<DD, CC, true><<<gkv, blk, 0, stream>>>(                    \
         (const bf16*)dout, (const bf16*)q, (const bf16*)k, (const bf16*)v,    \
         (const float*)lse, (const float*)delta, (float*)dk, (float*)dv, SQ,  \
@@ -639,7 +658,11 @@
                       int S, int D, float scale, int window,
                       const long* qstr, const long* kstr, const long* vstr,
                       const long* dostr, const int* q_start, const int* k_end,
-                      hipStream_t stream) {
+                      bool pipe, hipStream_t stream) {
+  if (pipe)
+    launch_flash_dkv_pipe(dout, q, k, v, lse, delta, dk, dv, B, HQ, HKV, S, S,
+                          D, true, scale, window, qstr, kstr, vstr, dostr, 2,
+                          q_start, k_end, stream);
   dim3 blk(512);
   dim3 gkv((S + 255) / 256, B * HQ);
   const bool small = ((long)((S + 255) / 256) * B * HQ) < 512;
@@ -647,6 +670,7 @@
   dim3 gq((S + bm - 1) / bm, B * HQ);
 #define CASE(DD)                                                              \
   do {                                                                        \
+    if (!pipe)                                                                \
     flash_bwd_dkv_kernel<DD, true, false, true><<<gkv, blk, 0, stream>>>(     \
         (const bf16*)dout, (const bf16*)q, (const bf16*)k, (const bf16*)v,    \
         (const float*)lse, (const float*)delta, (float*)dk, (float*)dv, S,   \
diff --git a/neuronx_distributed_training_amd/ops/csrc/flash_attn_bwd_dkv_pipe.hip b/neuronx_distributed_training_amd/ops/csrc/flash_attn_bwd_dkv_pipe.hip
--- /dev/null
+++ b/neuronx_distributed_training_amd/ops/csrc/flash_attn_bwd_dkv_pipe.hip
@@ -0,0 +1,344 @@
+#include "attn_common.h"
+
+template <int D, bool CAUSAL, bool RANGED = false, bool SEGMENTED = false>
+__global__ __launch_bounds__(512) void flash_bwd_dkv_pipe_kernel(
+    const bf16* __restrict__ dO, const bf16* __restrict__ Q,
+    const bf16* __restrict__ K, const bf16* __restrict__ V,
+    const float* __restrict__ LSE, const float* __restrict__ DELTA,
+    float* __restrict__ dK,
+    float* __restrict__ dV,
+    int SQ, int SKV, int Bb, int HQ, int HKV, float scale,
+    int window, long sQs, long sQb, long sQh, long sKs, long sKb, long sKh,
+    long sVs, long sVb, long sVh, long sDs, long sDb, long sDh,
+    const int* __restrict__ kv_lo = nullptr,
+    const int* __restrict__ kv_hi = nullptr) {
+  static_assert(!(RANGED && SEGMENTED), "one mask mode at a time");
+  static_assert(!SEGMENTED || CAUSAL, "segments are causal");
+  constexpr int BN = 256;
+  constexpr int BM = 64;
+  const int coff = SKV - SQ;
+  constexpr int KP = D + 8;
+  constexpr int VP = BM + 8;
+  __shared__ __attribute__((aligned(16))) __bf16 qdo_lds[2 * BM * KP];
+  __shared__ __attribute__((aligned(16))) __bf16 tr_lds[2 * D * VP];
+  __shared__ __attribute__((aligned(16))) __bf16 pds_lds[2 * 8 * 32 * VP];
+  __bf16* const q_lds = qdo_lds;
+  __bf16* const do_lds = qdo_lds + BM * KP;
+  __bf16* const dot_lds = tr_lds;
+  __bf16* const qt_lds = tr_lds + D * VP;
+  __bf16* const pT_lds = pds_lds;
+  __bf16* const dsT_lds = pds_lds + 8 * 32 * VP;
+  constexpr int PARK = (D == 128) ? 2 : 0;
+  __shared__ __attribute__((aligned(16))) __bf16 park_lds[PARK * 512 * 8 + 8];
+  __shared__ __attribute__((aligned(16))) float row_lds[3 * BM];
+
+  const int lane = threadIdx.x & 63;
+  const int wid = __builtin_amdgcn_readfirstlane(threadIdx.x >> 6);
+  const int group = HQ / HKV;
+  int kblock, bhg;
+  xcd_remap(kblock, bhg);
+  const int g = bhg % group;
+  const int hkv = (bhg / group) % HKV;
+  const int b = bhg / (group * HKV);
+  int lo = 0, hi = SKV;
+  if constexpr (RANGED) {
+    lo = kv_lo[b];
+    hi = kv_hi[b];
+  }
+
+  const bf16* Kp = K + b * sKb + hkv * sKh;
+  const bf16* Vp = V + b * sVb + hkv * sVh;
+  const int kbase = kblock * BN;
+  const int krow_w = kbase + wid * 32;
+
+  constexpr int DK = D / 32;
+  bf16x8_t kfrag[2][DK], vfrag[2][DK];
+#pragma unroll
+  for (int sb = 0; sb < 2; ++sb) {
+    const int r = krow_w + sb * 16 + (lane & 15);
+    const long row = (r < SKV) ? r : (SKV - 1);
+#pragma unroll
+    for (int kk = 0; kk < DK; ++kk) {
+      *(int4*)&kfrag[sb][kk] =
+          *(const int4*)(Kp + row * sKs + kk * 32 + (lane >> 4) * 8);
+      *(int4*)&vfrag[sb][kk] =
+          *(const int4*)(Vp + row * sVs + kk * 32 + (lane >> 4) * 8);
+#pragma unroll
+      for (int j = 0; j < 8; ++j)
+        kfrag[sb][kk][j] = (__bf16)((float)kfrag[sb][kk][j] * scale);
+    }
+  }
+
+#pragma unroll
+  for (int i = 0; i < PARK; ++i)
+    *(bf16x8_t*)&park_lds[(i * 512 + threadIdx.x) * 8] =
+        vfrag[1][DK - PARK + i];
+
+  constexpr int DN2 = D / 32;
+  f32x16_t dvacc[DN2], dkacc[DN2];
+#pragma unroll
+  for (int nj = 0; nj < DN2; ++nj) {
+    dvacc[nj] = f32x16_t{};
+    dkacc[nj] = f32x16_t{};
+  }
+
+  {
+    const int hq = hkv * group + g;
+    const bf16* Qp = Q + b * sQb + hq * sQh;
+    const bf16* dOp = dO + b * sDb + hq * sDh;
+    const float* Lp = LSE + ((long)b * HQ + hq) * SQ;
+    const float* Dp = DELTA + ((long)b * HQ + hq) * SQ;
+
+    const int klo = RANGED ? max(kbase, lo) : kbase;
+    const int khi = RANGED ? min(kbase + BN, hi) : kbase + BN;
+    const int ib0 = CAUSAL ? max(0, (klo - coff) / BM) : 0;
+    int nqb = (SQ + BM - 1) / BM;
+    if (CAUSAL && window > 0)
+      nqb = min(nqb, (khi - 1 + window - coff + BM - 1) / BM);
+    if (RANGED && klo >= khi) nqb = 0;
+    const int* Sp = kv_lo + (long)b * SQ;
+    if constexpr (SEGMENTED)
+      nqb = min(nqb,
+                (kv_hi[(long)b * SQ + min(kbase + BN, SKV) - 1] + BM - 1) / BM);
+
+    constexpr int C8 = D / 8;
+    const uint qrs = (uint)sQs * 2, dors = (uint)sDs * 2;
+    constexpr int NROWC = SEGMENTED ? 3 : 2;
+    const float* rowp = wid == 0 ? Lp : wid == 1 ? Dp : (const float*)Sp;
+
+    typedef int i32x4_t __attribute__((ext_vector_type(4)));
+    i32x4_t q0 = {0, 0, 0, 0}, q1 = q0, d0 = q0, d1 = q0;
+    float rowc = 0.f;
+    auto issue_tile = [&](int ib) {
+      const int qbase = ib * BM;
+      int t = threadIdx.x;
+      asm volatile("" : "+v"(t));
+      const int last = SQ - 1 - qbase;
+      if ((D == 128) || wid < 4) {
+        const int srow = (t / C8) * 2, scol = (t % C8) * 8;
+        const int r0 = min(srow, last), r1 = min(srow + 1, last);
+        const char* qt = (const char*)(Qp + (long)qbase * sQs);
+        const char* dt = (const char*)(dOp + (long)qbase * sDs);
+        q0 = *(const i32x4_t*)(qt + ((uint)r0 * qrs + scol * 2));
+        d0 = *(const i32x4_t*)(dt + ((uint)r0 * dors + scol * 2));
+        q1 = *(const i32x4_t*)(qt + ((uint)r1 * qrs + scol * 2));
+        d1 = *(const i32x4_t*)(dt + ((uint)r1 * dors + scol * 2));
+      }
+      if (wid < NROWC)
+        rowc = *(const float*)((const char*)(rowp + qbase) +
+                               (uint)min(t & 63, last) * 4);
+    };
+    auto write_tile = [&](int ib) {
+      asm volatile("" : "+v"(q0), "+v"(q1), "+v"(d0), "+v"(d1));
+      asm volatile("" : "+v"(rowc));
+      const int last = SQ - 1 - ib * BM;
+      int t = threadIdx.x;
+      asm volatile("" : "+v"(t));
+      if ((D == 128) || wid < 4) {
+        const int sr = (t / C8) * 2, sc = (t % C8) * 8;
+        if (sr > last) q0 = d0 = i32x4_t{0, 0, 0, 0};
+        if (sr + 1 > last) q1 = d1 = i32x4_t{0, 0, 0, 0};
+        *(i32x4_t*)&q_lds[sr * KP + sc] = q0;
+        *(i32x4_t*)&q_lds[(sr + 1) * KP + sc] = q1;
+        *(i32x4_t*)&do_lds[sr * KP + sc] = d0;
+        *(i32x4_t*)&do_lds[(sr + 1) * KP + sc] = d1;
+        const uint qw0[4] = {(uint)q0.x, (uint)q0.y, (uint)q0.z, (uint)q0.w};
+        const uint qw1[4] = {(uint)q1.x, (uint)q1.y, (uint)q1.z, (uint)q1.w};
+        const uint dw0[4] = {(uint)d0.x, (uint)d0.y, (uint)d0.z, (uint)d0.w};
+        const uint dw1[4] = {(uint)d1.x, (uint)d1.y, (uint)d1.z, (uint)d1.w};
+#pragma unroll
+        for (int j = 0; j < 8; ++j) {
+          const int m = j >> 1;
+          const uint qp = (j & 1) ? (qw0[m] >> 16) | (qw1[m] & 0xffff0000u)
+                                  : (qw0[m] & 0xffffu) | (qw1[m] << 16);
+          const uint dp = (j & 1) ? (dw0[m] >> 16) | (dw1[m] & 0xffff0000u)
+                                  : (dw0[m] & 0xffffu) | (dw1[m] << 16);
+          const int r = sc + j;
+          const uint byte = tr_swz((uint)(r * VP + sr) * 2, r);
+          *(uint*)((char*)qt_lds + byte) = qp;
+          *(uint*)((char*)dot_lds + byte) = dp;
+        }
+      }
+      if (wid < NROWC)
+        row_lds[wid * BM + (t & 63)] =
+            (t & 63) > last ? (wid == 0 ? 1e30f : 0.f) : rowc;
+    };
+
+    if (ib0 < nqb) issue_tile(ib0);
+    for (int ib = ib0; ib < nqb; ++ib) {
+      const int qbase = ib * BM;
+      write_tile(ib);
+      __syncthreads();
+      if (ib + 1 < nqb) issue_tile(ib + 1);
+
+      int qs_tile = 0;
+      if constexpr (SEGMENTED)
+        qs_tile = __builtin_amdgcn_readfirstlane(
+            __float_as_int(row_lds[2 * BM]));
+      if ((!CAUSAL || krow_w <= qbase + BM - 1 + coff) &&
+          (!RANGED || (krow_w < hi && krow_w + 32 > lo)) &&
+          (!SEGMENTED || krow_w + 32 > qs_tile)) {
+        __bf16* pw = &pT_lds[wid * 32 * VP];
+        __bf16* dw = &dsT_lds[wid * 32 * VP];
+        int ln = threadIdx.x;
+        asm volatile("" : "+v"(ln));
+        ln &= 63;
+        const int l15 = ln & 15;
+        const int lq = (ln >> 4) * 4;
+        const int dl = lq - l15;
+#pragma unroll
+        for (int nq = 0; nq < BM / 16; ++nq) {
+          f32x4_t st[2], dpt[2];
+          st[0] = st[1] = f32x4_t{0.f, 0.f, 0.f, 0.f};
+          dpt[0] = dpt[1] = f32x4_t{0.f, 0.f, 0.f, 0.f};
+#pragma unroll
+          for (int kk = 0; kk < DK; ++kk) {
+            bf16x8_t qa = load_frag_a(&q_lds[nq * 16 * KP], KP, kk * 32, ln);
+            st[0] = MFMA_16x16x32(qa, kfrag[0][kk], st[0]);
+            st[1] = MFMA_16x16x32(qa, kfrag[1][kk], st[1]);
+            bf16x8_t da = load_frag_a(&do_lds[nq * 16 * KP], KP, kk * 32, ln);
+            dpt[0] = MFMA_16x16x32(da, vfrag[0][kk], dpt[0]);
+            bf16x8_t vf1;
+            if (kk < DK - PARK)
+              vf1 = vfrag[1][kk];
+            else
+              vf1 = *(const bf16x8_t*)&park_lds[((kk - (DK - PARK)) * 512 +
+                                                 wid * 64 + ln) * 8];
+            dpt[1] = MFMA_16x16x32(da, vf1, dpt[1]);
+          }
+          __builtin_amdgcn_sched_barrier(0);
+          const f32x4_t lse = *(const f32x4_t*)&row_lds[nq * 16 + lq];
+          const f32x4_t delta = *(const f32x4_t*)&row_lds[BM + nq * 16 + lq];
+          bool full_patch =
+              (!RANGED || (krow_w >= lo && krow_w + 31 < hi)) &&
+              (qbase + nq * 16 + 15 < SQ) && (krow_w + 31 < SKV) &&
+              (!CAUSAL || (qbase + nq * 16 + coff >= krow_w + 31)) &&
+              (window <= 0 ||
+               (qbase + nq * 16 + 15 + coff < krow_w + window));
+          if constexpr (SEGMENTED)
+            full_patch = full_patch &&
+                         krow_w >= __builtin_amdgcn_readfirstlane(
+                                       __float_as_int(
+                                           row_lds[2 * BM + nq * 16 + 15]));
+          typedef __bf16 bf16x4_t __attribute__((ext_vector_type(4)));
+          if (full_patch) {
+#pragma unroll
+            for (int sb = 0; sb < 2; ++sb) {
+              bf16x4_t p4, ds4;
+#pragma unroll
+              for (int r = 0; r < 4; ++r) {
+                const float p = __expf(st[sb][r] - lse[r]);
+                const float ds = p * (dpt[sb][r] - delta[r]) * scale;
+                p4[r] = (__bf16)p;
+                ds4[r] = (__bf16)ds;
+              }
+              const int at = (sb * 16 + l15) * VP + nq * 16 + lq;
+              *(bf16x4_t*)&pw[at] = p4;
+              *(bf16x4_t*)&dw[at] = ds4;
+            }
+          } else {
+            const int q0 = qbase + nq * 16;
+            int qs[4] = {0, 0, 0, 0};
+            if constexpr (SEGMENTED) {
+              const int4 t = *(const int4*)&row_lds[2 * BM + nq * 16 + lq];
+              qs[0] = t.x, qs[1] = t.y, qs[2] = t.z, qs[3] = t.w;
+            }
+#pragma unroll
+            for (int sb = 0; sb < 2; ++sb) {
+              bf16x4_t p4, ds4;
+              const int k0 = krow_w + sb * 16;
+              const int kd = k0 - q0 - coff;
+              bool kdead = l15 >= SKV - k0;
+              if constexpr (RANGED) kdead |= (l15 < lo - k0) || (l15 >= hi - k0);
+#pragma unroll
+              for (int r = 0; r < 4; ++r) {
+                bool dead = kdead || (lq >= SQ - q0 - r) ||
+                            (CAUSAL && dl < kd - r);
+                if (CAUSAL && window > 0) dead |= (dl >= kd + window - r);
+                if constexpr (SEGMENTED) dead |= (l15 < qs[r] - k0);
+                const float p = dead ? 0.f : __expf(st[sb][r] - lse[r]);
+                const float ds = p * (dpt[sb][r] - delta[r]) * scale;
+                p4[r] = (__bf16)p;
+                ds4[r] = (__bf16)ds;
+              }
+              const int at = (sb * 16 + l15) * VP + nq * 16 + lq;
+              *(bf16x4_t*)&pw[at] = p4;
+              *(bf16x4_t*)&dw[at] = ds4;
+            }
+          }
+          __builtin_amdgcn_sched_barrier(0);
+        }
+        const int l31 = ln & 31;
+        const uint tra = (uint)(l31 * VP + (ln >> 5) * 8) * 2;
+        const uint trs = ((uint)(l31 >> 3) & 3u) << 4;
+#pragma unroll
+        for (int kq = 0; kq < BM / 16; ++kq) {
+          bf16x8_t pa = load_frag_a32(pw, VP, kq * 16, ln);
+          bf16x8_t da = load_frag_a32(dw, VP, kq * 16, ln);
+          const uint tr0 = (tra + kq * 32) ^ trs;
+          const uint tr1 = tr0 ^ 64u;
+#pragma unroll
+          for (int nj = 0; nj < DN2; ++nj) {
+            const uint byte = ((nj & 1) ? tr1 : tr0) + nj * 32 * VP * 2;
+            bf16x8_t dob, qb2;
+            *(int4*)&dob = *(const int4*)((const char*)dot_lds + byte);
+            dvacc[nj] = MFMA_32x32x16(pa, dob, dvacc[nj]);
+            *(int4*)&qb2 = *(const int4*)((const char*)qt_lds + byte);
+            dkacc[nj] = MFMA_32x32x16(da, qb2, dkacc[nj]);
+          }
+        }
+      }
+      __syncthreads();
+    }
+  }
+
+  const long sOs = (long)Bb * HKV * D;
+  const long slab = (long)g * SKV * sOs + ((long)b * HKV + hkv) * D;
+  float* dKp = dK + slab;
+  float* dVp = dV + slab;
+#pragma unroll
+  for (int nj = 0; nj < DN2; ++nj) {
+#pragma unroll
+    for (int r = 0; r < 16; ++r) {
+      const int krow = krow_w + (r & 3) + 8 * (r >> 2) + 4 * (lane >> 5);
+      if (krow < SKV) {
+        const int dcol = nj * 32 + (lane & 31);
+        dKp[(long)krow * sOs + dcol] = dkacc[nj][r];
+        dVp[(long)krow * sOs + dcol] = dvacc[nj][r];
+      }
+    }
+  }
+}
+
+extern "C" {
+void launch_flash_dkv_pipe(const void* dout, const void* q, const void* k,
+                           const void* v, const void* lse, const void* delta,
+                           void* dk, void* dv, int B, int HQ, int HKV, int SQ,
+                           int SKV, int D, bool causal, float scale,
+                           int window, const long* qstr, const long* kstr,
+                           const long* vstr, const long* dostr, int mode,
+                           const int* bound_a, const int* bound_b,
+                           hipStream_t stream) {
+  dim3 blk(512);
+  dim3 gkv((SKV + 255) / 256, B * HQ);
+#define CASE(DD, CC, RR, SS)                                                  \
+  flash_bwd_dkv_pipe_kernel<DD, CC, RR, SS><<<gkv, blk, 0, stream>>>(         \
+      (const bf16*)dout, (const bf16*)q, (const bf16*)k, (const bf16*)v,      \
+      (const float*)lse, (const float*)delta, (float*)dk, (float*)dv, SQ,    \
+      SKV, B, HQ, HKV, scale, window, qstr[0], qstr[1], qstr[2], kstr[0],     \
+      kstr[1], kstr[2], vstr[0], vstr[1], vstr[2], dostr[0], dostr[1],        \
+      dostr[2], bound_a, bound_b)
+#define CASE_D(DD)                                                            \
+  do {                                                                        \
+    if (mode == 2) CASE(DD, true, false, true);                               \
+    else if (mode == 1 && causal) CASE(DD, true, true, false);                \
+    else if (mode == 1) CASE(DD, false, true, false);                         \
+    else if (causal) CASE(DD, true, false, false);                            \
+    else CASE(DD, false, false, false);                                       \
+  } while (0)
+  if (D == 128) CASE_D(128);
+  else if (D == 64) CASE_D(64);
+#undef CASE_D
+#undef CASE
+}
+}
diff --git a/neuronx_distributed_training_amd/ops/flash_attn.py b/neuronx_distributed_training_amd/ops/flash_attn.py
--- a/neuronx_distributed_training_amd/ops/flash_attn.py
+++ b/neuronx_distributed_training_amd/ops/flash_attn.py
@@ -24,10 +24,22 @@
     return kern.flash_attn_fwd
 
 
+def _dkv_arm() -> str:
+    env = os.environ.get("NXDT_ATTN_DKV", "") or "pipe"
+    if env not in ("pipe", "sbuf"):
+        raise ValueError(f"NXDT_ATTN_DKV must be 'pipe' or 'sbuf', got {env!r}")
+    return env
+
+
+def v2_bwd_fn(kern, kind=""):
+    suffix = "_sbuf" if _dkv_arm() == "sbuf" else ""
+    return getattr(kern, f"flash_attn_bwd{kind}{suffix}")
+
+
 def _bwd_fn(kern, sq=None, skv=None):
     if _attn_version() == "3" and (sq is None or sq == skv):
         return kern.flash_attn_bwd_v3
-    return kern.flash_attn_bwd
+    return v2_bwd_fn(kern)
 
 
 def mask_to_kv_range_tensors(attention_mask):
@@ -185,12 +197,12 @@
             q, k, v, o, lse = ctx.saved_tensors
         kern = kernels_for(q)
         if kern is not None and ctx.segmented:
-            dq, dk, dv = kern.flash_attn_bwd_seg(
+            dq, dk, dv = v2_bwd_fn(kern, "_seg")(
                 do, q, k, v, o, lse, q_start, k_end, ctx.scale, ctx.window
             )
             return (dq, dk, dv) + none7
         if kern is not None and ctx.ranged:
-            dq, dk, dv = kern.flash_attn_bwd_range(
+            dq, dk, dv = v2_bwd_fn(kern, "_range")(
                 do, q, k, v, o, lse, kv_lo, kv_hi, ctx.causal, ctx.scale,
                 ctx.window,
             )
diff --git a/neuronx_distributed_training_amd/ops/ring_attn.py b/neuronx_distributed_training_amd/ops/ring_attn.py
--- a/neuronx_distributed_training_amd/ops/ring_attn.py
+++ b/neuronx_distributed_training_amd/ops/ring_attn.py
@@ -8,7 +8,7 @@
 import torch.distributed as dist
 
 from ..parallel import state as ps
-from .flash_attn import _FlashAttnFn, _cpu_ref_fwd, _make_mask
+from .flash_attn import _FlashAttnFn, _cpu_ref_fwd, _make_mask, v2_bwd_fn
 from . import kernels_for
 
 
@@ -68,7 +68,7 @@
 
 def _bwd_block(kern, do, q, k, v, out, lse, causal, scale):
     if kern is not None:
-        return kern.flash_attn_bwd(
+        return v2_bwd_fn(kern)(
             do.contiguous(), q, k, v, out, lse, causal, scale
         )
     return _cpu_block_bwd(do, q, k, v, out, lse, causal, scale)
diff --git a/setup.py b/setup.py
--- a/setup.py
+++ b/setup.py
@@ -23,6 +23,7 @@
         "flash_attn_fwd_v3.hip",
         "flash_attn_bwd_v3.hip",
         "flash_attn_bwd.hip",
+        "flash_attn_bwd_dkv_pipe.hip",
         "cross_entropy.hip",
         "moe_gemm.hip",
         "probe.hip",
```

After: 16940 tokens/s, median of 6. +7.3%, better.
